# domerin0/rnn-speech

Measured on AMD Instinct MI355X. Metric: audio_frames_per_sec_train_3x512_lstm_ctc, higher is better.
Workload: dtype f32

## Files before the change

### include/amdspeech.h

```cpp
#ifndef AMDSPEECH_H
#define AMDSPEECH_H

#include <stddef.h>
#include <stdint.h>

#ifdef __cplusplus
extern "C" {
#endif

#define AMDSPEECH_OK 0
#define AMDSPEECH_EINVAL (-1)
#define AMDSPEECH_EHIP (-2)
#define AMDSPEECH_EUNSUPPORTED (-3)
#define AMDSPEECH_ETIMEOUT (-4)

int amdspeech_version(void);
const char* amdspeech_last_error(void);
int amdspeech_device_cu_count(void);

int amdspeech_linear_fwd(void* stream, const float* x, const float* w, const float* b,
                         float* y, int M, int K, int N);
int amdspeech_linear_bwd(void* stream, const float* x, const float* w, const float* dy,
                         float* dx, float* dw, float* db, int M, int K, int N);

// ... 29 lines not shown
                               const float* A, int lda, const float* B, int ldb,
                               float* C, int ldc, const float* bias, int accumulate, void* scratch, size_t scratch_bytes);
int amdspeech_gemm_bf16_packed_plan(int transA, int transB, int M, int N, int K, int lda, int ldb, amdspeech_gemm_plan_info* out);
int amdspeech_bf16_copy(void* stream, const float* src, long ld, long rows, int cols, int transpose, unsigned short* dst, long ldd,
                        float* colsum, unsigned short* plain);
int amdspeech_bf16_transpose(void* stream, const unsigned short* src, long rows, int cols, unsigned short* dst, long ldd);

int amdspeech_batchnorm_fwd(void* stream, const float* x, float* y, float* xhat,
                            float* inv_std, int T, int B, int H, float eps);
int amdspeech_batchnorm_bwd(void* stream, const float* dy, const float* xhat,
                            const float* inv_std, float* dx, int T, int B, int H);

int amdspeech_batchnorm_sum(void* stream, const float* x, const float* global_sum, int n_total, float* out,
                            int T, int B, int H);
int amdspeech_batchnorm_apply(void* stream, const float* x, const float* global_sum, const float* global_sq,
                              int n_total, float eps, float* y, float* xhat, float* inv_std, int T, int B, int H);
int amdspeech_batchnorm_bwd_sums(void* stream, const float* dy, const float* xhat, float* sums, int T, int B, int H);
int amdspeech_batchnorm_bwd_apply(void* stream, const float* dy, const float* xhat, const float* inv_std,
                                  const float* global_sums, int n_total, float* dx, int T, int B, int H);

typedef struct amdspeech_lstm_desc {
    int T, B, H, L;
    float keep_in, keep_out;
    uint64_t seed;
    int precision;
    int flags;
} amdspeech_lstm_desc;

enum { AMDSPEECH_LSTM_ARMED = 1, AMDSPEECH_LSTM_ARM_NEXT = 2, AMDSPEECH_LSTM_SAME_WS = 4, AMDSPEECH_LSTM_PER_DIAGONAL = 8,
       AMDSPEECH_LSTM_INJECT_TIMEOUT = 16 };

enum {
    AMDSPEECH_LSTM_WS_Z0 = 0,
    AMDSPEECH_LSTM_WS_ZTOP = 1,
    AMDSPEECH_LSTM_WS_DZTOP = 2,
    AMDSPEECH_LSTM_WS_DZ0 = 3,
    AMDSPEECH_LSTM_WS_HFINAL = 4,
    AMDSPEECH_LSTM_WS_CFINAL = 5,
    AMDSPEECH_LSTM_WS_GATES = 6
};
size_t amdspeech_lstm_workspace_bytes(const amdspeech_lstm_desc* d);
void* amdspeech_lstm_ws_ptr(const amdspeech_lstm_desc* d, void* ws, int which);

int amdspeech_lstm_workspace_release(void* stream, void* ws);

int amdspeech_lstm_beside_forward(void* stream, const void* ws);

int amdspeech_lstm_beside_tail(void* stream, const void* ws);

int amdspeech_lstm_fwd(void* stream, const amdspeech_lstm_desc* d, void* ws,
                       const float* kernels, long kernel_stride,
                       const float* biases, long bias_stride,
                       const int* lengths, const float* h0, const float* c0);
int amdspeech_lstm_pair_fusable(const amdspeech_lstm_desc* d);
int amdspeech_lstm_fwd_pair(void* stream, const amdspeech_lstm_desc* d_a, void* ws_a, const float* kernels_a, const float* biases_a,
                            const amdspeech_lstm_desc* d_b, void* ws_b, const float* kernels_b, const float* biases_b,
                            long kernel_stride, long bias_stride, const int* lengths, const float* h0_a, const float* c0_a);
int amdspeech_lstm_bwd_pair(void* stream, const amdspeech_lstm_desc* d_a, void* ws_a, const float* kernels_a, float* dkernels_a, float* dbiases_a,
                            const amdspeech_lstm_desc* d_b, void* ws_b, const float* kernels_b, float* dkernels_b, float* dbiases_b,
                            long kernel_stride, long bias_stride, const int* lengths);
int amdspeech_lstm_status(const amdspeech_lstm_desc* d, void* ws);
int amdspeech_lstm_bwd(void* stream, const amdspeech_lstm_desc* d, void* ws,
                       const float* kernels, long kernel_stride,
                       float* dkernels, float* dbiases, long bias_stride,
                       const int* lengths);

typedef struct amdspeech_ctc_head {
    const float* w_out;
    const float* b_out;
    float* logits;
    const int* dense_labels;
    float* loss;
    float* dlogits;
    void* ctc_ws;
    int C, U;
} amdspeech_ctc_head;
int amdspeech_lstm_ctc_fusable(const amdspeech_lstm_desc* d, int C, int U);
int amdspeech_lstm_fwd_ctc(void* stream, const amdspeech_lstm_desc* d, void* ws,
                           const float* kernels, long kernel_stride, const float* biases, long bias_stride,
                           const int* lengths, const float* h0, const float* c0, const amdspeech_ctc_head* head);
int amdspeech_lstm_bwd_ctc(void* stream, const amdspeech_lstm_desc* d, void* ws,
                           const float* kernels, long kernel_stride, float* dkernels, float* dbiases, long bias_stride,
                           const int* lengths, const amdspeech_ctc_head* head);

int amdspeech_lstm_dropout_multipliers(void* stream, const amdspeech_lstm_desc* d, int which, int layer, float* out);

enum { AMDSPEECH_LSTM_PATH_FLOW = 0, AMDSPEECH_LSTM_PATH_BIG1 = 1, AMDSPEECH_LSTM_PATH_BIG = 2, AMDSPEECH_LSTM_PATH_HOIST = 3,
       AMDSPEECH_LSTM_PATH_DIAG = 4, AMDSPEECH_LSTM_PATH_DIAG_BF3 = 5 };
typedef struct amdspeech_lstm_plan_info {
    int fwd_path, bwd_path, nmt, kb, mv, wpx, uw, fwd_mt, pair, bf16p, bf16p_reserved, xw_parts, nfw, w_pieces, dz0_inkernel, flow2_q;
} amdspeech_lstm_plan_info;
int amdspeech_lstm_plan(const amdspeech_lstm_desc* d, int C, int U, amdspeech_lstm_plan_info* out);
int amdspeech_lstm_plan_xw_halves(const amdspeech_lstm_desc* d, int C, int U);
int amdspeech_lstm_plan_xw_ksteps(const amdspeech_lstm_desc* d, int C, int U);

enum {
    AMDSPEECH_BIDIR_WS_Z0 = 0, AMDSPEECH_BIDIR_WS_YTOP_FW = 1, AMDSPEECH_BIDIR_WS_YTOP_BW = 2, AMDSPEECH_BIDIR_WS_DYTOP_FW = 3,
    AMDSPEECH_BIDIR_WS_DYTOP_BW = 4, AMDSPEECH_BIDIR_WS_DZ0 = 5, AMDSPEECH_BIDIR_WS_HFINAL = 6, AMDSPEECH_BIDIR_WS_CFINAL = 7
};
size_t amdspeech_lstm_bidir_workspace_bytes(const amdspeech_lstm_desc* d);
void* amdspeech_lstm_bidir_ws_ptr(const amdspeech_lstm_desc* d, void* ws, int which);
long amdspeech_lstm_bidir_layer_stride(const amdspeech_lstm_desc* d);
int amdspeech_lstm_bidir_path(const amdspeech_lstm_desc* d);
typedef struct amdspeech_lstm_bidir_plan_info {
    int path, cus, fwd_kpw, fwd_waves, fwd_groups, fwd_wgs, fwd_lds, bwd_kpw, bwd_waves, bwd_groups, bwd_wgs, bwd_lds;
} amdspeech_lstm_bidir_plan_info;
int amdspeech_lstm_bidir_plan(const amdspeech_lstm_desc* d, amdspeech_lstm_bidir_plan_info* out);
int amdspeech_lstm_bidir_fwd(void* stream, const amdspeech_lstm_desc* d, void* ws, const float* const* kernels,
                             const float* const* biases, const int* lengths, const float* h0, const float* c0);
int amdspeech_lstm_bidir_bwd(void* stream, const amdspeech_lstm_desc* d, void* ws, const float* const* kernels,
                             float* const* dkernels, float* const* dbiases, const int* lengths);
int amdspeech_lstm_bidir_status(const amdspeech_lstm_desc* d, void* ws);
int amdspeech_lstm_bidir_dropout_multipliers(void* stream, const amdspeech_lstm_desc* d, int dir, int which, int layer, float* out);

size_t amdspeech_ctc_workspace_bytes(int T, int B, int C, int U);
int amdspeech_ctc_loss_fwd_bwd(void* stream, const float* logits, const int* dense_labels,
                               const int* lengths, int T, int B, int C, int U,
                               float* loss, float* dlogits, void* ws);
int amdspeech_ctc_loss_fwd_bwd_staged(void* stream, const float* logits, const int* dense_labels,
                                      const int* lengths, int T, int B, int C, int U, float* loss,
                                      float* dlogits, void* ws, int stage);

enum { AMDSPEECH_CTC_KERNEL_WAVE = 0, AMDSPEECH_CTC_KERNEL_SHIFT = 1, AMDSPEECH_CTC_KERNEL_PAIR = 2, AMDSPEECH_CTC_KERNEL_EDGE = 3 };
typedef struct amdspeech_ctc_plan_info {
    int kernel, threads, rmax, smax;
} amdspeech_ctc_plan_info;
int amdspeech_ctc_plan(int T, int B, int C, int U, amdspeech_ctc_plan_info* out);

size_t amdspeech_ctc_align_workspace_bytes(int T, int B, int C, int U);
int amdspeech_ctc_align_plan(int T, int B, int C, int U, amdspeech_ctc_plan_info* out);
int amdspeech_ctc_align(void* stream, const float* logits, const int* dense_labels, const int* lengths,
                        int T, int B, int C, int U, int* frame_label, int* frame_state, int* spans,
                        float* score, float* confidence, void* ws);

int amdspeech_ctc_greedy_decode(void* stream, const float* logits, const int* lengths,
                                int T, int B, int C, int* ids, int* out_len, int* ws);

int amdspeech_merge_repeated(void* stream, int* ids, int* lens, int T, int B, int pad);

int amdspeech_edit_distance(void* stream, const int* a, const int* a_len, int lda, const int* b,
                            const int* b_len, int ldb, int n_pairs, int* out);

int amdspeech_ctc_beam_search_host(const float* logits, const int* lengths, int T, int B, int C,
                                   int beam_width, int merge_repeated, int* ids, int* out_len,
                                   float* log_prob);
int amdspeech_ctc_beam_search_host_mt(const float* logits, const int* lengths, int T, int B, int C,
                                      int beam_width, int merge_repeated, int* ids, int* out_len,
                                      float* log_prob, int max_threads);
int amdspeech_ctc_beam_search_host_nbest(const float* logits, const int* lengths, int T, int B, int C,
                                         int beam_width, int merge_repeated, int n_best, int* ids, int* out_len,
                                         float* log_prob, int* n_found, int max_threads);

int amdspeech_edit_distance_host(const int* a, const int* a_len, int lda, const int* b, const int* b_len, int ldb,
                                 int n_pairs, int* out);

uint32_t amdspeech_crc32c(const void* data, size_t n, uint32_t crc);

int amdspeech_audio_probe(const char* path, int* sample_rate, int* channels, long* frames);
int amdspeech_audio_decode(const char* path, float* out, long capacity, long* frames, int* sample_rate,
                           int verify);

size_t amdspeech_resample_workspace_bytes(int B);
int amdspeech_resample_num_samples(int n_samples, int rate_in, int rate_out);
int amdspeech_resample(void* stream, const float* pcm, const int* n_samples, int B, int n_max, int rate_in,
                       int rate_out, float* out, int out_max, void* ws);

// ... 149 lines not shown
```

### rnn-speech_amd/csrc/common.h

```cpp
#pragma once
#include <hip/hip_runtime.h>
#include <stdint.h>
#include <stdio.h>
#include <stdarg.h>
#include <mutex>

#include "../../include/amdspeech.h"

namespace amdspeech {

void set_error(const char* fmt, ...);

#define AS_CHECK_ARG(cond, ...)                         \
    do {                                                \
        if (!(cond)) {                                  \
            ::amdspeech::set_error(__VA_ARGS__);        \
            return AMDSPEECH_EINVAL;                    \
        }                                               \
    } while (0)

#define AS_CHECK_HIP(expr)                                                          \
    do {                                                                            \
        hipError_t e__ = (expr);                                                    \
        if (e__ != hipSuccess) {                                                    \
// ... 20 lines not shown
        first = (__atomic_load_n(seen, __ATOMIC_ACQUIRE) & bit) == 0;
    }
    explicit operator bool() const { return first; }
    void done() { if (bit) __atomic_fetch_or(seen, bit, __ATOMIC_RELEASE); }
};

int runtime_switch(const char* name, int dflt);
#ifdef AMDSPEECH_DEVTRACE
static inline int dev_knob(const char* name, int dflt) { return runtime_switch(name, dflt); }
const char* dev_knob_str(const char* name);
#else
static inline int dev_knob(const char*, int dflt) { return dflt; }
static inline const char* dev_knob_str(const char*) { return nullptr; }
#endif

static inline int ceil_div(long a, long b) { return (int)((a + b - 1) / b); }
static inline size_t align_up(size_t x, size_t a) { return (x + a - 1) / a * a; }

typedef float f32x4 __attribute__((ext_vector_type(4)));
typedef float f32x16 __attribute__((ext_vector_type(16)));

int gemm_f32(hipStream_t s, bool transA, bool transB, int M, int N, int K, const float* A, int lda,
             const float* B, int ldb, float* C, int ldc, const float* bias, bool accumulate,
             float* colsum = nullptr,
             const int* gate = nullptr, int gate_need = 0,
             unsigned* gate_err = nullptr);
typedef amdspeech_gemm_plan_info GemmPlan;
int gemm_f32_plan(bool transA, bool transB, int M, int N, int K, const float* A, int lda, const float* B, int ldb, const float* C,
                  int ldc, const float* bias, bool accumulate, bool colsum, bool gate, GemmPlan* out);
int gemm_f32_launch(hipStream_t s, const GemmPlan& p, bool transA, bool transB, int M, int N, int K, const float* A, int lda,
                    const float* B, int ldb, float* C, int ldc, const float* bias, bool accumulate, float* colsum = nullptr,
                    const int* gate = nullptr, int gate_need = 0, unsigned* gate_err = nullptr);
bool gemm_skinny_plan(bool transB, int M, int N, int K, const float* A, int lda, const float* B, int ldb, const float* C, int ldc,
                      const float* bias, GemmPlan* out);
int gemm_skinny_launch(hipStream_t s, const GemmPlan& p, bool transB, int M, int N, int K, const float* A, int lda, const float* B,
                       int ldb, float* C, int ldc, const float* bias, bool accumulate);
bool gemm_skinny_tn_plan(int M, int N, int K, const float* A, int lda, const float* B, int ldb, bool accumulate, bool colsum, GemmPlan* out);
int gemm_skinny_tn_launch(hipStream_t s, const GemmPlan& p, int M, int N, int K, const float* A, int lda, const float* B, int ldb,
                          float* C, int ldc, bool accumulate, float* colsum);
constexpr int GEMM_GROUP_MAX = AMDSPEECH_GEMM_GROUP_MAX;
int gemm_f32_tn_group(hipStream_t s, int count, int M, int N, int K, const float* const* A, int lda, const float* const* B,
                      int ldb, float* const* C, int ldc, float* const* colsum, bool accumulate,
                      const int* gate = nullptr, int gate_need = 0, unsigned* gate_err = nullptr);
bool gemm_f32_tn_group_ok(int M, int N, int K, const float* A, int lda, const float* B, int ldb);
int gemm_f32_tn_group_plan(int count, int M, int N, int K, const float* A, int lda, const float* B, int ldb, const float* C,
                           bool accumulate, GemmPlan* out);
int colsum_accumulate(hipStream_t s, const float* x, int rows, int cols, int ld, float* out);
int gemm_bf3(hipStream_t s, bool transA, bool transB, int M, int N, int K, const float* A, int lda, const float* B, int ldb,
             float* C, int ldc, const float* bias, bool accumulate);
int gemm_bf16(hipStream_t s, bool transA, bool transB, int M, int N, int K, const float* A, int lda, const float* B, int ldb,
              float* C, int ldc, const float* bias, bool accumulate);
int gemm_bf_plan(bool single, bool transA, bool transB, int M, int N, int K, const float* A, int lda, const float* B, int ldb,
                 const float* C, int ldc, const float* bias, bool accumulate, GemmPlan* out);

int bf16p_copy(hipStream_t s, const float* src, long ld, long rows, int cols, bool transpose, unsigned short* dst, long ldd, float* colsum,
               unsigned short* plain = nullptr);
size_t bf16p_partial_bytes(int M, int N, int K);
size_t bf16p_partial_bytes_max();
int bf16p_transpose(hipStream_t s, const unsigned short* src, long rows, int cols, unsigned short* dst, long ldd);
int bf16p_gemm(hipStream_t s, int M, int N, int K, const unsigned short* Ak, long lda, const unsigned short* Bk, long ldb, float* C, long ldc,
               const float* bias, bool accumulate, void* partial, size_t partial_bytes);
bool gemm_bf16_packed_ok(bool transA, bool transB, int M, int N, int K, int lda, int ldb);
size_t gemm_bf16_packed_scratch_bytes(int M, int N, int K);
int gemm_bf16_packed(hipStream_t s, bool transA, bool transB, int M, int N, int K, const float* A, int lda, const float* B, int ldb,
                     float* C, int ldc, const float* bias, bool accumulate, float* colsum, void* scratch, size_t scratch_bytes);

int ctc_prepare_targets(hipStream_t s, const int* dense_labels, const int* lengths, int T, int B, int C, int U, void* ws);

__host__ __device__ __forceinline__ uint32_t mix32(uint32_t x) {
    x ^= x >> 16; x *= 0x7feb352dU; x ^= x >> 15; x *= 0x846ca68bU; x ^= x >> 16;
    return x;
}
__device__ __forceinline__ float uniform01(uint64_t seed, uint32_t tensor, uint32_t idx) {
    uint32_t a = mix32(idx ^ (uint32_t)seed);
    uint32_t b = mix32(a + tensor * 0x9e3779b9U + (uint32_t)(seed >> 32));
    return (float)(b >> 8) * (1.0f / 16777216.0f);
}
__host__ __device__ __forceinline__ uint32_t random24(uint64_t seed, uint32_t stream, uint32_t idx) {
    uint32_t a = mix32(idx ^ (uint32_t)seed);
    uint32_t b = mix32(a + stream * 0x9e3779b9U + (uint32_t)(seed >> 32));
    return b >> 8;
}

}
```

### rnn-speech_amd/csrc/gemm_skinny.hip

```cpp
#include "common.h"
#include <string.h>

namespace amdspeech {

typedef __amdgpu_buffer_rsrc_t sk_rsrc_t;
typedef unsigned sk_u32x4 __attribute__((ext_vector_type(4)));

struct SkinnyArgs {
    const float* A; const float* B; float* C; const float* bias;
    int M, N, K, lda, ldb, ldc, accumulate;
};

constexpr unsigned SK_OOB = 0x80000000u;

__device__ __forceinline__ f32x4 sk_load4(sk_rsrc_t rs, unsigned byte_off) {
    const sk_u32x4 w = __builtin_amdgcn_raw_buffer_load_b128(rs, byte_off, 0, 0);
    f32x4 r;
    r.x = __uint_as_float(w.x); r.y = __uint_as_float(w.y); r.z = __uint_as_float(w.z); r.w = __uint_as_float(w.w);
    return r;
}
__device__ __forceinline__ float sk_load1(sk_rsrc_t rs, unsigned byte_off) {
    return __uint_as_float(__builtin_amdgcn_raw_buffer_load_b32(rs, byte_off, 0, 0));
}

struct SkinnyOut {
    sk_rsrc_t c, c_in, bias;
    __device__ __forceinline__ void init(const SkinnyArgs& g) {
        const unsigned cbytes = (unsigned)(((size_t)(g.M - 1) * g.ldc + g.N) * 4);
        c = __builtin_amdgcn_make_buffer_rsrc(g.C, 0, cbytes, 0x00020000);
        c_in = __builtin_amdgcn_make_buffer_rsrc(g.C, 0, g.accumulate ? cbytes : 0u, 0x00020000);
        bias = __builtin_amdgcn_make_buffer_rsrc(const_cast<float*>(g.bias), 0, g.bias != nullptr ? (unsigned)g.N * 4u : 0u, 0x00020000);
    }
    __device__ __forceinline__ unsigned offset(const SkinnyArgs& g, int row, int n) const {
        return (row < g.M && n < g.N) ? (unsigned)((size_t)row * g.ldc + n) * 4u : SK_OOB;
    }
    __device__ __forceinline__ f32x4 addend(const SkinnyArgs& g, unsigned off, int n) const {
        return sk_load4(bias, n < g.N ? (unsigned)n * 4u : SK_OOB) + sk_load4(c_in, off);
    }
    __device__ __forceinline__ void store(unsigned off, f32x4 v) const {
        sk_u32x4 w;
        w.x = __float_as_uint(v.x); w.y = __float_as_uint(v.y); w.z = __float_as_uint(v.z); w.w = __float_as_uint(v.w);
        __builtin_amdgcn_raw_buffer_store_b128(w, c, off, 0, 0);
    }
};

template <int NT>
__global__ __launch_bounds__(256) void gemm_skinny_n_kernel(SkinnyArgs g) {
    constexpr int KC = 64, LD = NT * 16 + ((NT & 1) ? 4 : 12);
    static_assert((4 * LD) % 32 == 16 && LD % 4 == 0, "bank spread");
    __shared__ __attribute__((aligned(16))) float wt[2][KC][LD];
    const int tid = threadIdx.x, w = tid >> 6, lane = tid & 63, m = lane & 15, kg = lane >> 4;
    const int row = blockIdx.x * 64 + w * 16 + m;
    const sk_rsrc_t ra = __builtin_amdgcn_make_buffer_rsrc(const_cast<float*>(g.A), 0, (unsigned)(((size_t)(g.M - 1) * g.lda + g.K) * 4), 0x00020000);
    const sk_rsrc_t rb = __builtin_amdgcn_make_buffer_rsrc(const_cast<float*>(g.B), 0, (unsigned)(((size_t)(g.K - 1) * g.ldb + g.N) * 4), 0x00020000);
    const int chunks = (g.K + KC - 1) / KC;

    f32x4 wreg[NT], a_cur[4], a_nxt[4];
    auto load_w = [&](int c) __attribute__((always_inline)) {
#pragma unroll
        for (int i = 0; i < NT; ++i) {
            const int slot = i * 256 + tid, k = slot / (4 * NT), n4 = slot % (4 * NT);
            const int kk = c * KC + k;
            const bool ok = n4 * 4 < g.N && kk < g.K;
            wreg[i] = sk_load4(rb, ok ? (unsigned)(kk * g.ldb + n4 * 4) * 4u : SK_OOB);
        }
    };
    auto put_w = [&](int buf) __attribute__((always_inline)) {
#pragma unroll
        for (int i = 0; i < NT; ++i) {
            const int slot = i * 256 + tid, k = slot / (4 * NT), n4 = slot % (4 * NT);
            *reinterpret_cast<f32x4*>(&wt[buf][k][n4 * 4]) = wreg[i];
        }
    };
    auto load_a = [&](int c, f32x4* a) __attribute__((always_inline)) {
#pragma unroll
        for (int s = 0; s < 4; ++s) {
            const int kk = c * KC + 16 * s + 4 * kg;
            const bool ok = row < g.M && kk < g.K;
            a[s] = sk_load4(ra, ok ? (unsigned)((size_t)row * g.lda + kk) * 4u : SK_OOB);
        }
    };

    f32x4 acc[NT];
#pragma unroll
    for (int i = 0; i < NT; ++i) acc[i] = f32x4{0.f, 0.f, 0.f, 0.f};
    load_w(0);
    load_a(0, a_cur);
    put_w(0);
    __syncthreads();
    for (int c = 0; c < chunks; ++c) {
        const int buf = c & 1;
        load_w(c + 1);
        load_a(c + 1, a_nxt);
        __builtin_amdgcn_sched_barrier(0);
        float bq[2][NT][4];
        auto read_b = [&](int s, float (*b)[4]) __attribute__((always_inline)) {
#pragma unroll
            for (int nt = 0; nt < NT; ++nt) {
                const float* col = &wt[buf][16 * s + 4 * kg][nt * 16 + m];
                b[nt][0] = col[0]; b[nt][1] = col[LD]; b[nt][2] = col[2 * LD]; b[nt][3] = col[3 * LD];
            }
        };
        read_b(0, bq[0]);
#pragma unroll
        for (int s = 0; s < 4; ++s) {
            if (s < 3) read_b(s + 1, bq[(s + 1) & 1]);
            __builtin_amdgcn_sched_barrier(0);
#pragma unroll
            for (int j = 0; j < 4; ++j)
#pragma unroll
                for (int nt = 0; nt < NT; ++nt)
                    acc[nt] = __builtin_amdgcn_mfma_f32_16x16x4f32(bq[s & 1][nt][j], a_cur[s][j], acc[nt], 0, 0, 0);
            __builtin_amdgcn_sched_barrier(0);
        }
        put_w(buf ^ 1);
#pragma unroll
        for (int s = 0; s < 4; ++s) a_cur[s] = a_nxt[s];
        __syncthreads();
    }
    SkinnyOut out;
    out.init(g);
    unsigned off[NT];
    f32x4 add[NT];
#pragma unroll
    for (int nt = 0; nt < NT; ++nt) {
        off[nt] = out.offset(g, row, nt * 16 + 4 * kg);
        add[nt] = out.addend(g, off[nt], nt * 16 + 4 * kg);
    }
#pragma unroll
    for (int nt = 0; nt < NT; ++nt) out.store(off[nt], acc[nt] + add[nt]);
}

template <int KT, bool B_KC>
__global__ __launch_bounds__(256) void gemm_skinny_k_kernel(SkinnyArgs g) {
    const int tid = threadIdx.x, w = tid >> 6, lane = tid & 63, m = lane & 15, kg = lane >> 4;
    const int row0 = blockIdx.x * 128 + w * 32;
    const sk_rsrc_t ra = __builtin_amdgcn_make_buffer_rsrc(const_cast<float*>(g.A), 0, (unsigned)(((size_t)(g.M - 1) * g.lda + g.K) * 4), 0x00020000);
    const size_t b_extent = B_KC ? (size_t)(g.N - 1) * g.ldb + g.K : (size_t)(g.K - 1) * g.ldb + g.N;
    const sk_rsrc_t rb = __builtin_amdgcn_make_buffer_rsrc(const_cast<float*>(g.B), 0, (unsigned)(b_extent * 4), 0x00020000);
    SkinnyOut out;
    out.init(g);

    f32x4 a[2][KT];
#pragma unroll
    for (int mt = 0; mt < 2; ++mt)
#pragma unroll
        for (int kt = 0; kt < KT; ++kt) {
            const int row = row0 + mt * 16 + m, kk = 16 * kt + 4 * kg;
            const bool ok = row < g.M && kk < g.K;
            a[mt][kt] = sk_load4(ra, ok ? (unsigned)((size_t)row * g.lda + kk) * 4u : SK_OOB);
        }
    struct Tile { f32x4 b[2][KT], bias[2], old[2][2]; unsigned off[2][2]; };
    auto fetch = [&](int nt, Tile& t) __attribute__((always_inline)) {
#pragma unroll
        for (int q = 0; q < 2; ++q) {
            const int n = (nt + q) * 16 + m;
#pragma unroll
            for (int kt = 0; kt < KT; ++kt) {
                const int kk = 16 * kt + 4 * kg;
                const bool ok = n < g.N && kk < g.K;
                if (B_KC) {
                    t.b[q][kt] = sk_load4(rb, ok ? (unsigned)(n * g.ldb + kk) * 4u : SK_OOB);
                } else {
                    const unsigned o = ok ? (unsigned)(kk * g.ldb + n) * 4u : SK_OOB;
                    const unsigned st = ok ? (unsigned)g.ldb * 4u : 0u;
                    t.b[q][kt].x = sk_load1(rb, o);
                    t.b[q][kt].y = sk_load1(rb, o + st);
                    t.b[q][kt].z = sk_load1(rb, o + 2 * st);
                    t.b[q][kt].w = sk_load1(rb, o + 3 * st);
                }
            }
            const int nc = (nt + q) * 16 + 4 * kg;
            t.bias[q] = sk_load4(out.bias, nc < g.N ? (unsigned)nc * 4u : SK_OOB);
#pragma unroll
            for (int mt = 0; mt < 2; ++mt) {
                t.off[mt][q] = out.offset(g, row0 + mt * 16 + m, nc);
                t.old[mt][q] = sk_load4(out.c_in, t.off[mt][q]);
            }
        }
    };
    auto tile = [&](int nt, const Tile& cur, Tile& nxt) __attribute__((always_inline)) {
        fetch(nt + 2, nxt);
        __builtin_amdgcn_sched_barrier(0);
        f32x4 acc[2][2];
#pragma unroll
        for (int mt = 0; mt < 2; ++mt)
#pragma unroll
            for (int q = 0; q < 2; ++q) acc[mt][q] = cur.bias[q] + cur.old[mt][q];
#pragma unroll
        for (int kt = 0; kt < KT; ++kt)
#pragma unroll
            for (int j = 0; j < 4; ++j)
#pragma unroll
                for (int mt = 0; mt < 2; ++mt)
#pragma unroll
                    for (int q = 0; q < 2; ++q)
                        acc[mt][q] = __builtin_amdgcn_mfma_f32_16x16x4f32(cur.b[q][kt][j], a[mt][kt][j], acc[mt][q], 0, 0, 0);
#pragma unroll
        for (int mt = 0; mt < 2; ++mt)
#pragma unroll
            for (int q = 0; q < 2; ++q) out.store(cur.off[mt][q], acc[mt][q]);
        __builtin_amdgcn_sched_barrier(0);
    };
    const int all_tiles = (g.N + 15) / 16;
    const int per = ((all_tiles + (int)gridDim.y - 1) / (int)gridDim.y + 1) & ~1;
    const int nt0 = (int)blockIdx.y * per, ntiles = min(all_tiles, nt0 + per);
    Tile t0, t1;
    fetch(nt0, t0);
    for (int nt = nt0; nt < ntiles; nt += 4) {
        tile(nt, t0, t1);
        if (nt + 2 >= ntiles) break;
        tile(nt + 2, t1, t0);
    }
}

#ifndef SKTN_DIAG
#define SKTN_DIAG 0
#endif
struct SkinnyTnArgs {
    const float* S; const float* W; float* C; float* colsum;
    int K, s, wide, lds, ldw, ldc;
    int chunk;
    int nslices;
    int small_is_a;
    int colsum_small;
};

template <int FULL, int RT>
__global__ __launch_bounds__(512) void gemm_skinny_tn_kernel(SkinnyTnArgs g) {
    constexpr int NTS = 4 * FULL + RT;
    constexpr int PD = NTS <= 4 ? 4 : 2;
    constexpr int SP = 64 * FULL + 16 * RT, LDR = 65;
    constexpr int NF = FULL > 0 ? FULL : 1, NR = RT > 0 ? RT : 1;
    extern __shared__ __attribute__((aligned(16))) float lds[];
    const int tid = threadIdx.x, w = tid >> 6, lane = tid & 63, i = lane & 15, kq = lane >> 4;
    const int v = blockIdx.x, xcd = v & 7, q = v >> 3;
    const int chunk_id = xcd + 8 * (q / g.nslices), slice = q % g.nslices;
    const int r0 = chunk_id * g.chunk;
    if (r0 >= g.K) return;
    const sk_rsrc_t rs = __builtin_amdgcn_make_buffer_rsrc(const_cast<float*>(g.S), 0, (unsigned)(((size_t)(g.K - 1) * g.lds + g.s) * 4), 0x00020000);
    const sk_rsrc_t rw = __builtin_amdgcn_make_buffer_rsrc(const_cast<float*>(g.W), 0, (unsigned)(((size_t)(g.K - 1) * g.ldw + g.wide) * 4), 0x00020000);

    const int wcol = slice * 64 + 4 * i;
    const bool w_ok = wcol < g.wide;
    const bool ones_wanted = g.colsum != nullptr && !g.colsum_small;
    const int rem = g.s - 64 * FULL;
    const int rcol = 64 * FULL + RT * i;
    bool r_valid[NR];
#pragma unroll
    for (int e = 0; e < NR; ++e) r_valid[e] = RT > 0 && rcol + e < g.s;
    const bool ones_lane = ones_wanted && RT > 0 && i == rem / NR;
    const int ones_e = rem % NR;
    const bool cs_small = g.colsum != nullptr && g.colsum_small && slice == 0;
    const int groups = g.chunk / 32;
    f32x4 smf[PD][NF], wd[PD];
    float smr[PD][NR];
    auto fetch = [&](int t, int p) __attribute__((always_inline)) {
        const int row = r0 + 4 * (8 * t + w) + kq;
        const bool r_ok = row < g.K && t < groups;
        wd[p] = sk_load4(rw, (r_ok && w_ok) ? (unsigned)((size_t)row * g.ldw + wcol) * 4u : SK_OOB);
#pragma unroll
        for (int b = 0; b < FULL; ++b) smf[p][b] = sk_load4(rs, r_ok ? (unsigned)((size_t)row * g.lds + 64 * b + 4 * i) * 4u : SK_OOB);
        if (RT > 0) {
            const unsigned off = (r_ok && r_valid[0]) ? (unsigned)((size_t)row * g.lds + rcol) * 4u : SK_OOB;
            if (RT == 1) {
                smr[p][0] = sk_load1(rs, off);
            } else if (RT == 2) {
                typedef unsigned u2 __attribute__((ext_vector_type(2)));
                const u2 x = __builtin_amdgcn_raw_buffer_load_b64(rs, off, 0, 0);
                smr[p][0] = __uint_as_float(x.x); smr[p][1 % NR] = __uint_as_float(x.y);
            } else if (RT == 3) {
                typedef unsigned u3 __attribute__((ext_vector_type(3)));
                const u3 x = __builtin_amdgcn_raw_buffer_load_b96(rs, off, 0, 0);
                smr[p][0] = __uint_as_float(x.x); smr[p][1 % NR] = __uint_as_float(x.y); smr[p][2 % NR] = __uint_as_float(x.z);
            } else {
                const f32x4 x = sk_load4(rs, off);
                smr[p][0] = x.x; smr[p][1 % NR] = x.y; smr[p][2 % NR] = x.z; smr[p][3 % NR] = x.w;
            }
        }
    };
// ... 183 lines not shown
    g.colsum_small = small_is_a ? 0 : 1;
    g.nslices = p.tiles_n;
    g.chunk = p.k_chunk;
    if (p.zero_fill) {
        const long n = (long)M * N;
        hipLaunchKernelGGL(skinny_zero_kernel, dim3(ceil_div(n, 256)), dim3(256), 0, st, C, M, N, ldc);
    }
    const dim3 grid(p.grid), block(512);
    const int full = p.variant / 8, rt = p.variant % 8;
    const size_t lds = (size_t)2 * (4 * full + rt) * 4 * 64 * 16;
#define SK_TN(F, R)                                                                                                          \
    do {                                                                                                                      \
        static unsigned long long seen = 0;                                                                                   \
        if (DeviceOnce once{&seen}) {                                                                                         \
            AS_CHECK_HIP(hipFuncSetAttribute(reinterpret_cast<const void*>(gemm_skinny_tn_kernel<F, R>),                      \
                                             hipFuncAttributeMaxDynamicSharedMemorySize, 2 * (4 * F + R) * 4 * 64 * 16));      \
            once.done();                                                                                                      \
        }                                                                                                                     \
        hipLaunchKernelGGL((gemm_skinny_tn_kernel<F, R>), grid, block, lds, st, g);                                           \
    } while (0)
    switch (p.variant) {
        case 1: SK_TN(0, 1); break;
        case 2: SK_TN(0, 2); break;
        case 3: SK_TN(0, 3); break;
        case 4: SK_TN(0, 4); break;
        case 8: SK_TN(1, 0); break;
        case 9: SK_TN(1, 1); break;
        case 10: SK_TN(1, 2); break;
        case 11: SK_TN(1, 3); break;
        case 12: SK_TN(1, 4); break;
        default: AS_CHECK_ARG(false, "gemm_skinny_tn: no kernel for variant %d", p.variant);
    }
#undef SK_TN
    AS_CHECK_LAUNCH();
    return AMDSPEECH_OK;
}

bool gemm_skinny_plan(bool transB, int M, int N, int K, const float* A, int lda, const float* B, int ldb, const float* C, int ldc,
                      const float* bias, GemmPlan* out) {
    static const bool enabled = dev_knob("AMDSPEECH_GEMM_SKINNY", 1) != 0;
    if (!enabled || M < 256) return false;
    if ((N | K | lda | ldb | ldc) & 3) return false;
    if (!aligned16(A) || !aligned16(B) || !aligned16(C) || (bias != nullptr && !aligned16(bias))) return false;
    const size_t lim = (size_t)SK_OOB;
    if (((size_t)(M - 1) * lda + K) * 4 >= lim) return false;
    if (((size_t)(M - 1) * ldc + N) * 4 >= lim) return false;
    GemmPlan p;
    memset(&p, 0, sizeof(p));
    p.splits = 1; p.col_slices = 1; p.k_chunk = K; p.a_vec = p.b_vec = 1; p.tiles_n = 1;
    if (K <= 80 && N >= 64) {
        const size_t be = transB ? (size_t)(N - 1) * ldb + K : (size_t)(K - 1) * ldb + N;
        if (be * 4 >= lim) return false;
        const int row_blocks = ceil_div(M, 128);
        const int kt = ceil_div(K, 16);
        p.family = AMDSPEECH_GEMM_SKINNY_K; p.variant = (kt <= 3 ? 3 : 5) * 2 + (transB ? 1 : 0);
        p.tiles_m = row_blocks;
        p.col_slices = (row_blocks < 512 && N >= 256 && kt <= 3) ? 2 : 1;
        p.grid = row_blocks * p.col_slices;
        *out = p;
        return true;
    }
    if (!transB && N <= 96 && K >= 64) {
        if (((size_t)(K - 1) * ldb + N) * 4 >= lim) return false;
        const int nt = ceil_div(N, 16);
        p.family = AMDSPEECH_GEMM_SKINNY_N; p.variant = nt < 6 ? nt : 6;
        p.tiles_m = ceil_div(M, 64);
        p.grid = p.tiles_m;
        *out = p;
        return true;
    }
    return false;
}

int gemm_skinny_launch(hipStream_t s, const GemmPlan& p, bool transB, int M, int N, int K, const float* A, int lda, const float* B,
                       int ldb, float* C, int ldc, const float* bias, bool accumulate) {
    SkinnyArgs g;
    g.A = A; g.B = B; g.C = C; g.bias = bias; g.M = M; g.N = N; g.K = K; g.lda = lda; g.ldb = ldb; g.ldc = ldc;
    g.accumulate = accumulate ? 1 : 0;
    const dim3 block(256);
    if (p.family == AMDSPEECH_GEMM_SKINNY_K) {
        const dim3 grid(p.tiles_m, p.col_slices);
#define SK_K(KT)                                                                                           \
        do {                                                                                               \
            if (transB) hipLaunchKernelGGL((gemm_skinny_k_kernel<KT, true>), grid, block, 0, s, g);        \
            else hipLaunchKernelGGL((gemm_skinny_k_kernel<KT, false>), grid, block, 0, s, g);              \
        } while (0)
        if (p.variant / 2 == 3) SK_K(3);
        else SK_K(5);
#undef SK_K
    } else {
        const dim3 grid(p.grid);
        switch (p.variant) {
            case 1: hipLaunchKernelGGL(gemm_skinny_n_kernel<1>, grid, block, 0, s, g); break;
            case 2: hipLaunchKernelGGL(gemm_skinny_n_kernel<2>, grid, block, 0, s, g); break;
            case 3: hipLaunchKernelGGL(gemm_skinny_n_kernel<3>, grid, block, 0, s, g); break;
            case 4: hipLaunchKernelGGL(gemm_skinny_n_kernel<4>, grid, block, 0, s, g); break;
            case 5: hipLaunchKernelGGL(gemm_skinny_n_kernel<5>, grid, block, 0, s, g); break;
            default: hipLaunchKernelGGL(gemm_skinny_n_kernel<6>, grid, block, 0, s, g); break;
        }
    }
    AS_CHECK_LAUNCH();
    return AMDSPEECH_OK;
}

}
```

### rnn-speech_amd/csrc/lstm.hip

```cpp
#include "common.h"
#include "gemm_core.h"
#include "ctc_core.h"
#include <stdlib.h>
#include <string.h>
#include <type_traits>
#include <mutex>
#include <unordered_map>

namespace amdspeech {

#define FLOW_WEIGHTS_RESIDENT() __builtin_amdgcn_s_waitcnt(0x0F70)
static unsigned long long* dev_trace_ptr() {
#ifdef AMDSPEECH_DEVTRACE
    if (const char* e = dev_knob_str("AMDSPEECH_TRACE_PTR")) return reinterpret_cast<unsigned long long*>(strtoull(e, nullptr, 0));
#endif
    return nullptr;
}
#ifndef BIG_WEIGHTS_RESIDENT
#define BIG_WEIGHTS_RESIDENT 1
#endif

struct LstmLayout {
    size_t wp, wq, z, hs, cs, gates, dg, dztop, dz0, dc, xp0, xp, hp, dgp, sync, xph, hph, dxh, prec, pdown, xwp, bigring, wopack, bfs, total;
    size_t fwd_set = 0;
// ... 19 lines not shown
    const long groups = (long)d->L * ((d->B + 15) / 16);
    return fwd_workers_fit(d) && fwd_worker_wgs_per_xcd(d, 4) <= 32 - FWD2_WORKER_RESERVE &&
           (size_t)d->T * groups * (d->H / 16) * 6144 < (1ull << 32);
}
static bool bf16p_layout_reserved(const amdspeech_lstm_desc* d) {
    static const int env = runtime_switch("AMDSPEECH_BF16_PACKED", 1);
    return env != 0 && d->precision == 2 && d->H == 1024;
}
static bool bf16p_layout_on(const amdspeech_lstm_desc* d) {
    return bf16p_layout_reserved(d) && ((long)d->T * d->B) % 64 == 0 && (long)d->T * d->B >= 256;
}
struct Bf16pBufs { unsigned short *zb, *wtb, *dgb, *wb, *zht, *dgt; char* partial; size_t partial_bytes; };
static size_t bf16p_scratch_floats(const amdspeech_lstm_desc* d) {
    const size_t TB = ((size_t)d->T * d->B + 63) / 64 * 64, H = d->H;
    const size_t bytes = TB * H * 2 + 4 * H * H * 2 + TB * 4 * H * 2 + H * 4 * H * 2 + 2 * H * TB * 2 + 4 * H * TB * 2 +
                         bf16p_partial_bytes_max() + 8 * 256;
    return (bytes + 3) / 4;
}
static Bf16pBufs bf16p_bufs(const amdspeech_lstm_desc* d, float* base) {
    const size_t TB = (size_t)d->T * d->B, H = d->H;
    char* p = reinterpret_cast<char*>(base);
    auto take = [&](size_t bytes) { char* r = p; p += align_up(bytes, 256); return r; };
    Bf16pBufs b;
    b.zb = reinterpret_cast<unsigned short*>(take(TB * H * 2));
    b.wtb = reinterpret_cast<unsigned short*>(take(4 * H * H * 2));
    b.dgb = reinterpret_cast<unsigned short*>(take(TB * 4 * H * 2));
    b.wb = reinterpret_cast<unsigned short*>(take(H * 4 * H * 2));
    b.zht = reinterpret_cast<unsigned short*>(take(2 * H * TB * 2));
    b.dgt = reinterpret_cast<unsigned short*>(take(4 * H * TB * 2));
    b.partial_bytes = bf16p_partial_bytes_max();
    b.partial = take(b.partial_bytes);
    return b;
}
static int bf16p_xw(hipStream_t s, const Bf16pBufs& b, int rows, int H, const float* Z, const float* K, float* G, const float* bias) {
    if (int rc = bf16p_copy(s, Z, H, rows, H, false, b.zb, H, nullptr)) return rc;
    if (int rc = bf16p_copy(s, K, 4 * H, H, 4 * H, true, b.wtb, H, nullptr)) return rc;
    return bf16p_gemm(s, rows, 4 * H, H, b.zb, H, b.wtb, H, G, 4 * H, bias, false, b.partial, b.partial_bytes);
}
static int bf16p_dx(hipStream_t s, const Bf16pBufs& b, int rows, int H, const float* dG, const float* K, float* dX) {
    if (int rc = bf16p_copy(s, dG, 4 * H, rows, 4 * H, false, b.dgb, 4 * H, nullptr)) return rc;
    if (int rc = bf16p_copy(s, K, 4 * H, H, 4 * H, false, b.wb, 4 * H, nullptr)) return rc;
    return bf16p_gemm(s, rows, H, 4 * H, b.dgb, 4 * H, b.wb, 4 * H, dX, H, nullptr, false, b.partial, b.partial_bytes);
}
static int bf16p_layer_bwd(hipStream_t s, const Bf16pBufs& b, int rows, int H, const float* Z, const float* Hp, const float* dG, const float* K,
                           float* dX, float* dK, float* dbias) {
    if (int rc = bf16p_copy(s, dG, 4 * H, rows, 4 * H, true, b.dgt, rows, dbias, b.dgb)) return rc;
    if (int rc = bf16p_copy(s, K, 4 * H, H, 4 * H, false, b.wb, 4 * H, nullptr)) return rc;
    if (int rc = bf16p_gemm(s, rows, H, 4 * H, b.dgb, 4 * H, b.wb, 4 * H, dX, H, nullptr, false, b.partial, b.partial_bytes)) return rc;
    if (int rc = bf16p_copy(s, Z, H, rows, H, true, b.zht, rows, nullptr)) return rc;
    if (int rc = bf16p_copy(s, Hp, H, rows, H, true, b.zht + (size_t)H * rows, rows, nullptr)) return rc;
    return bf16p_gemm(s, 2 * H, 4 * H, rows, b.zht, rows, b.dgt, rows, dK, 4 * H, nullptr, true, b.partial, b.partial_bytes);
}
static int bf16p_layer_bwd_copied(hipStream_t s, const Bf16pBufs& b, int rows, int H, const float* Z, const float* Hp, const float* K,
                                  float* dX, float* dK) {
    if (int rc = bf16p_copy(s, K, 4 * H, H, 4 * H, false, b.wb, 4 * H, nullptr)) return rc;
    if (int rc = bf16p_gemm(s, rows, H, 4 * H, b.dgb, 4 * H, b.wb, 4 * H, dX, H, nullptr, false, b.partial, b.partial_bytes)) return rc;
    if (int rc = bf16p_copy(s, Z, H, rows, H, true, b.zht, rows, nullptr)) return rc;
    if (int rc = bf16p_copy(s, Hp, H, rows, H, true, b.zht + (size_t)H * rows, rows, nullptr)) return rc;
    if (int rc = bf16p_transpose(s, b.dgb, rows, 4 * H, b.dgt, rows)) return rc;
    return bf16p_gemm(s, 2 * H, 4 * H, rows, b.zht, rows, b.dgt, rows, dK, 4 * H, nullptr, true, b.partial, b.partial_bytes);
}
static int bf16p_dk(hipStream_t s, const Bf16pBufs& b, int rows, int H, const float* Z, const float* Hp, const float* dG, float* dK, float* dbias) {
    if (int rc = bf16p_copy(s, Z, H, rows, H, true, b.zht, rows, nullptr)) return rc;
    if (int rc = bf16p_copy(s, Hp, H, rows, H, true, b.zht + (size_t)H * rows, rows, nullptr)) return rc;
    if (int rc = bf16p_copy(s, dG, 4 * H, rows, 4 * H, true, b.dgt, rows, dbias)) return rc;
    return bf16p_gemm(s, 2 * H, 4 * H, rows, b.zht, rows, b.dgt, rows, dK, 4 * H, nullptr, true, b.partial, b.partial_bytes);
}

static int check_desc(const amdspeech_lstm_desc* d) {
    AS_CHECK_ARG(d != nullptr, "lstm: null descriptor");
    AS_CHECK_ARG(d->T > 0 && d->B > 0 && d->H > 0 && d->L > 0, "lstm: bad shape T=%d B=%d H=%d L=%d",
                 d->T, d->B, d->H, d->L);
    AS_CHECK_ARG(d->H % 16 == 0, "lstm: hidden size %d must be a multiple of 16", d->H);
    AS_CHECK_ARG(d->keep_in > 0.f && d->keep_in <= 1.f && d->keep_out > 0.f && d->keep_out <= 1.f,
                 "lstm: keep probabilities must be in (0,1]");
    AS_CHECK_ARG((size_t)d->T * d->B * d->H < (1ull << 32), "lstm: T*B*H too large for the dropout counter");
    AS_CHECK_ARG(d->precision == 0 || ((d->precision == 1 || d->precision == 2) && d->H % 32 == 0),
                 "lstm: precision %d unsupported (0 = f32; 1 = bf16x3, 2 = bf16: both need H %% 32 == 0, H = %d)", d->precision, d->H);
    AS_CHECK_ARG((d->flags & ~(AMDSPEECH_LSTM_ARMED | AMDSPEECH_LSTM_ARM_NEXT | AMDSPEECH_LSTM_SAME_WS | AMDSPEECH_LSTM_PER_DIAGONAL |
                               AMDSPEECH_LSTM_INJECT_TIMEOUT)) == 0, "lstm: unknown flags 0x%x", d->flags);
    return AMDSPEECH_OK;
}

struct DropCfg { float keep_in, keep_out; uint64_t seed; int L; };

__device__ __forceinline__ float zmult(const DropCfg& c, int lp, uint32_t idx) {
    float m = 1.0f;
    if (c.keep_in < 1.0f && lp < c.L)
        m *= (uniform01(c.seed, 2u * lp, idx) < c.keep_in) ? (1.0f / c.keep_in) : 0.0f;
    if (c.keep_out < 1.0f && lp >= 1)
        m *= (uniform01(c.seed, 2u * (lp - 1) + 1u, idx) < c.keep_out) ? (1.0f / c.keep_out) : 0.0f;
    return m;
}

__global__ void apply_zmult_kernel(float* x, long n, DropCfg c, int lp) {
    long i = (long)blockIdx.x * blockDim.x + threadIdx.x;
    if (i < n) x[i] *= zmult(c, lp, (uint32_t)i);
}

__global__ void pack_fwd_kernel(const float* __restrict__ kernels, long kstride, float* __restrict__ wp,
                                int H, int L, int UW, int grouped) {
    const int NT = UW / 4, NKB = 2 * H / 16, NUB = H / UW;
    const long total = (long)L * 2 * H * 4 * H;
    long o = (long)blockIdx.x * blockDim.x + threadIdx.x;
    if (o >= total) return;
    int m = o & 3, lane = (o >> 2) & 63;
    long r = o >> 8;
    int nt = r % NT; r /= NT;
    int kb = r % NKB; r /= NKB;
    int ub = r % NUB; int l = r / NUB;
    int j = lane & 15, kq = lane >> 4;
    int c = nt * 16 + j, g = c / UW, u = c % UW;
    if (grouped) { g = j >> 2; u = nt * 4 + (j & 3); }
    int k = kb * 16 + 4 * kq + m;
    wp[o] = kernels[l * kstride + (long)k * 4 * H + g * H + ub * UW + u];
}

__global__ void pack_bwd_kernel(const float* __restrict__ kernels, long kstride, float* __restrict__ wq,
                                int H, int L) {
    const int NRB = 2 * H / 16, NKB = 4 * H / 16;
    const long total = (long)L * 2 * H * 4 * H;
    long o = (long)blockIdx.x * blockDim.x + threadIdx.x;
    if (o >= total) return;
    int m = o & 3, lane = (o >> 2) & 63;
    long r = o >> 8;
    int kb = r % NKB; r /= NKB;
    int rb = r % NRB; int l = r / NRB;
    int row = rb * 16 + (lane & 15), col = kb * 16 + 4 * (lane >> 4) + m;
    wq[o] = kernels[l * kstride + (long)row * 4 * H + col];
}

__device__ __forceinline__ size_t packed_off(int row, int k, int K) {
    return ((((size_t)(row >> 4) * (K >> 4) + (k >> 4)) * 64) + (((k >> 2) & 3) * 16 + (row & 15))) * 4 + (k & 3);
}

__global__ void pack_rows_kernel(const float* __restrict__ src, size_t src_stride, float* __restrict__ dst,
                                 int B, int K, int nmat) {
    const size_t per = (size_t)B * K;
    const size_t i = (size_t)blockIdx.x * blockDim.x + threadIdx.x;
    if (i >= per * nmat) return;
    const int mat = i / per;
    const size_t r = i % per;
    const int row = r / K, k = r % K;
    const size_t bpk = (size_t)((B + 15) / 16 * 16) * K;
    dst[(size_t)mat * bpk + packed_off(row, k, K)] = src[(size_t)mat * src_stride + r];
}

__global__ __launch_bounds__(256) void mask_pack_rows_kernel(float* __restrict__ z, float* __restrict__ dst, int B, int K, int T,
                                                             DropCfg c, int masked) {
    const size_t per4 = (size_t)B * K / 4;
    const size_t i = (size_t)blockIdx.x * blockDim.x + threadIdx.x;
    if (i >= per4 * T) return;
    const int t = i / per4;
    const size_t r = (i % per4) * 4;
    const int row = r / K, k = r % K;
    const size_t e = (size_t)t * B * K + r;
    float4 v = *reinterpret_cast<const float4*>(z + e);
    if (masked) {
        v.x *= zmult(c, 0, (uint32_t)e); v.y *= zmult(c, 0, (uint32_t)(e + 1));
        v.z *= zmult(c, 0, (uint32_t)(e + 2)); v.w *= zmult(c, 0, (uint32_t)(e + 3));
        *reinterpret_cast<float4*>(z + e) = v;
    }
    const size_t bpk = (size_t)((B + 15) / 16 * 16) * K;
    *reinterpret_cast<float4*>(dst + (size_t)t * bpk + packed_off(row, k, K)) = v;
}

__global__ __launch_bounds__(256) void flow_fwd_prepare_kernel(const float* __restrict__ h0, const float* __restrict__ c0,
                                                               float* __restrict__ hs, float* __restrict__ cs,
                                                               float* __restrict__ hph, unsigned* __restrict__ sync_words,
                                                               int T, int B, int H, int L) {
    const int bp = (B + 15) / 16 * 16;
    const size_t per = (size_t)bp * H;
    const size_t i = (size_t)blockIdx.x * blockDim.x + threadIdx.x;
    if (i < 40) sync_words[i] = 0u;
    if (i >= per * L) return;
    const int l = i / per;
    const size_t r = i % per;
    const int row = r / H, k = r % H;
    float hv = 0.f;
    if (row < B) {
        const size_t e = (size_t)row * H + k, bh = (size_t)B * H;
        hv = h0 ? h0[l * bh + e] : 0.f;
        hs[(size_t)l * (T + 1) * bh + e] = hv;
        cs[(size_t)l * (T + 1) * bh + e] = c0 ? c0[l * bh + e] : 0.f;
    }
    hph[(size_t)l * (T + 1) * per + packed_off(row, k, H)] = hv;
}

__device__ __forceinline__ float sigmoidf_(float x) { return 1.0f / (1.0f + expf(-x)); }

#include "lstm_step_fwd.h"
#include "lstm_flow.h"
}
#include "ctc_flow.h"
namespace amdspeech {

#include "lstm_flow_fwd.h"
#include "lstm_big_fwd.h"
#include "lstm_step_bwd.h"
#include "lstm_flow_bwd.h"
#include "lstm_big_bwd.h"
#include "lstm_step_bf3.h"
constexpr int PROF_SEGS = 16;
static bool g_prof_on = false;
static hipEvent_t g_prof_ev[2][PROF_SEGS][2];
static int g_prof_launches[2] = {0, 0};
static int g_prof_nseg[2] = {0, 0};
static bool g_prof_valid[2] = {false, false};
static double g_prof_flops[2][2] = {{0, 0}, {0, 0}};
static void prof_flops(int which, double recurrence, double other) { g_prof_flops[which][0] = recurrence; g_prof_flops[which][1] = other; }

static void prof_begin(int which, hipStream_t s, int seg = 0) {
    if (g_prof_on && seg < PROF_SEGS) (void)hipEventRecord(g_prof_ev[which][seg][0], s);
}
static void prof_end(int which, hipStream_t s, int launches, int seg = 0) {
    if (!g_prof_on || seg >= PROF_SEGS) return;
    (void)hipEventRecord(g_prof_ev[which][seg][1], s);
    g_prof_launches[which] = launches;
    g_prof_nseg[which] = seg + 1;
    g_prof_valid[which] = true;
}

static hipStream_t g_side = nullptr;
static hipEvent_t g_fork = nullptr;
static int side_stream_init() {
    if (g_side) return AMDSPEECH_OK;
    AS_CHECK_HIP(hipStreamCreateWithFlags(&g_side, hipStreamNonBlocking));
    AS_CHECK_HIP(hipEventCreateWithFlags(&g_fork, hipEventDisableTiming));
    return AMDSPEECH_OK;
}
static hipStream_t g_chain = nullptr, g_gemm = nullptr;
static hipEvent_t g_ev_a = nullptr, g_ev_b = nullptr, g_ev_c = nullptr;
static int g_overlap_state = 0;
static int overlap_init() {
    if (g_overlap_state != 0) return g_overlap_state;
    g_overlap_state = -1;
    int dev = 0, cus = 0;
    if (hipGetDevice(&dev) != hipSuccess) return -1;
    if (hipDeviceGetAttribute(&cus, hipDeviceAttributeMultiprocessorCount, dev) != hipSuccess || cus != 256) return -1;
    uint32_t chain_mask[8] = {0, 0, ~0u, ~0u, ~0u, ~0u, ~0u, ~0u}, gemm_mask[8] = {~0u, ~0u, 0, 0, 0, 0, 0, 0};
    if (hipExtStreamCreateWithCUMask(&g_chain, 8, chain_mask) != hipSuccess) return -1;
    if (hipExtStreamCreateWithCUMask(&g_gemm, 8, gemm_mask) != hipSuccess) return -1;
    if (hipEventCreateWithFlags(&g_ev_a, hipEventDisableTiming) != hipSuccess) return -1;
    if (hipEventCreateWithFlags(&g_ev_b, hipEventDisableTiming) != hipSuccess) return -1;
    if (hipEventCreateWithFlags(&g_ev_c, hipEventDisableTiming) != hipSuccess) return -1;
    g_overlap_state = 1;
    return 1;
}
constexpr int DK_CHUNKS = 8, DK_SIDE = 5;

static int gemm_reduced(const amdspeech_lstm_desc* d, hipStream_t s, bool ta, bool tb, int M, int N, int K, const float* A, int lda,
                        const float* B, int ldb, float* C, int ldc, const float* bias, bool accumulate) {
    return (d->precision == 2 ? gemm_bf16 : gemm_bf3)(s, ta, tb, M, N, K, A, lda, B, ldb, C, ldc, bias, accumulate);
}
static int gemm_batched(const amdspeech_lstm_desc* d, hipStream_t s, bool ta, bool tb, int M, int N, int K, const float* A, int lda,
                        const float* B, int ldb, float* C, int ldc, const float* bias, bool accumulate) {
    if (d->precision != 0) return gemm_reduced(d, s, ta, tb, M, N, K, A, lda, B, ldb, C, ldc, bias, accumulate);
    return gemm_f32(s, ta, tb, M, N, K, A, lda, B, ldb, C, ldc, bias, accumulate);
}
static int pick_uw(const amdspeech_lstm_desc* d) {
    const long wgs8 = (long)d->L * (d->H / 8) * ceil_div(d->B, 32);
    return (d->H % 8 == 0 && wgs8 >= 96) ? 8 : 4;
}

static int device_cus() {
    static int cus = -1;
    if (cus < 0) {
        int dev = 0;
        if (hipGetDevice(&dev) != hipSuccess ||
            hipDeviceGetAttribute(&cus, hipDeviceAttributeMultiprocessorCount, dev) != hipSuccess) cus = 0;
    }
    return cus;
}

static bool use_big_fwd(const amdspeech_lstm_desc* d) {
    static const int env = runtime_switch("AMDSPEECH_BIG", 1);
    return env != 0 && !(d->flags & AMDSPEECH_LSTM_PER_DIAGONAL) && d->precision >= 0 && d->precision <= 2 && d->H == 1024 &&
           (d->B + 15) / 16 <= 4 && device_cus() == 256 &&
           (size_t)2 * ((d->B + 15) / 16 * 16) * d->H * 4 < (1ull << 32);
}

static bool use_flow(const amdspeech_lstm_desc* d) {
    static const int env = runtime_switch("AMDSPEECH_FLOW", 1);
    return env != 0 && !(d->flags & AMDSPEECH_LSTM_PER_DIAGONAL) && flow_shape_ok(d) && device_cus() == 256 && d->L * ((d->B + 15) / 16) <= 8;
}

template <bool CF>
static void (*flow_fwd_kernel(int kb, int pr, int mv, int mh, int me))(FlowArgs) {
    switch (kb) {
        case 1: return lstm_fwd_flow2<1, 0, 0, CF>;
        case 2: return pr == 2 ? lstm_fwd_flow2<2, 2, 0, CF> : (pr == 1 ? lstm_fwd_flow2<2, 1, 0, CF> : lstm_fwd_flow2<2, 0, 0, CF>);
        case 3: return lstm_fwd_flow2<3, 0, 0, CF>;
        default:
            if (pr == 0 && mv == 1 && mh == 1) return me > 0 ? lstm_fwd_flow2<4, 0, 1, CF, 1, FWD2_HALF_KSTEPS> : lstm_fwd_flow2<4, 0, 1, CF, 1>;
            if (pr == 0 && mv == 1) return lstm_fwd_flow2<4, 0, 1, CF>;
            return pr == 2 ? lstm_fwd_flow2<4, 2, 0, CF> : (pr == 1 ? lstm_fwd_flow2<4, 1, 0, CF> : lstm_fwd_flow2<4, 0, 0, CF>);
    }
}
template <bool CF>
static void (*flow_bwd_kernel(int kb, int pr))(FlowBwdArgs) {
    if (pr == 2) return kb == 2 ? lstm_bwd_flow2<2, 2, CF> : lstm_bwd_flow2<4, 2, CF>;
    if (pr == 1) return kb == 2 ? lstm_bwd_flow2<2, 1, CF> : lstm_bwd_flow2<4, 1, CF>;
    return kb == 1 ? lstm_bwd_flow2<1, 0, CF> : (kb == 2 ? lstm_bwd_flow2<2, 0, CF> : (kb == 3 ? lstm_bwd_flow2<3, 0, CF> : lstm_bwd_flow2<4, 0, CF>));
}
static int flow_fill_fwd_panels(hipStream_t s, const amdspeech_lstm_desc* d, float* ws, const LstmLayout& lo, int set) {
    const size_t bph = (size_t)(d->B + 15) / 16 * 16 * d->H;
    float* base = ws + (size_t)set * lo.fwd_set;
    AS_CHECK_HIP(hipMemsetD32Async(reinterpret_cast<hipDeviceptr_t>(base + lo.xph + (size_t)d->T * bph), (int)FLOW_SENTINEL,
                                   (size_t)d->L * d->T * bph, s));
    AS_CHECK_HIP(hipMemsetD32Async(reinterpret_cast<hipDeviceptr_t>(base + lo.hph), (int)FLOW_SENTINEL, (size_t)d->L * (d->T + 1) * bph, s));
    return AMDSPEECH_OK;
}
static int flow_fill_bwd_panels(hipStream_t s, const amdspeech_lstm_desc* d, float* ws, const LstmLayout& lo, bool ctc_head = false) {
    const size_t bpg = (size_t)((d->B + 15) / 16) * 16 * 4 * d->H;
    AS_CHECK_HIP(hipMemsetAsync(ws + lo.prec, 0, (lo.total - lo.prec) * sizeof(float), s));
    if (ctc_head)
        AS_CHECK_HIP(hipMemsetD32Async(reinterpret_cast<hipDeviceptr_t>(ws + lo.dztop), (int)FLOW_SENTINEL, (size_t)d->T * d->B * d->H, s));
    if (d->L > 1)
        AS_CHECK_HIP(hipMemsetD32Async(reinterpret_cast<hipDeviceptr_t>(ws + lo.dxh), (int)FLOW_SENTINEL,
                                       (size_t)(d->L - 1) * d->T * (bpg / 4), s));
    return AMDSPEECH_OK;
}
struct ArmState {
    hipEvent_t join = nullptr; bool pending = false;
    hipEvent_t pre = nullptr; int idle_xcds = 0;
    hipEvent_t post = nullptr; int post_flags = 0;
    int clean_set = 0;
    int xw_par = -1;
    int xw_cover = 0;
    long xw_key = 0;
};
static std::mutex g_arm_mutex;
static std::unordered_map<const void*, ArmState> g_arm;
static int flow_xw_parity(hipStream_t s, const void* ws, bool trust, long key, float* xwp, size_t frame_floats, int T, unsigned* par) {
    std::lock_guard<std::mutex> lock(g_arm_mutex);
    ArmState& st = g_arm[ws];
    if (trust && st.xw_par >= 0 && st.xw_key == key) {
        const int old = st.xw_par;
        if (T > st.xw_cover)
            AS_CHECK_HIP(hipMemsetD32Async(reinterpret_cast<hipDeviceptr_t>(xwp + (size_t)st.xw_cover * frame_floats), old,
                                           (size_t)(T - st.xw_cover) * frame_floats, s));
        st.xw_par = old ^ 1;
    } else {
        AS_CHECK_HIP(hipMemsetAsync(xwp, 0, (size_t)T * frame_floats * sizeof(float), s));
        st.xw_par = 1;
    }
    st.xw_cover = T; st.xw_key = key;
    *par = (unsigned)st.xw_par;
    return AMDSPEECH_OK;
}
static void flow_xw_forget(const void* ws) {
    std::lock_guard<std::mutex> lock(g_arm_mutex);
    auto it = g_arm.find(ws);
    if (it != g_arm.end()) it->second.xw_par = -1;
}
static int flow_arm_fork(hipStream_t s) {
    if (int rc = side_stream_init()) return rc;
    AS_CHECK_HIP(hipEventRecord(g_fork, s));
    AS_CHECK_HIP(hipStreamWaitEvent(g_side, g_fork, 0));
    return AMDSPEECH_OK;
}
static int flow_clean_set(const void* ws) {
    std::lock_guard<std::mutex> lock(g_arm_mutex);
    auto it = g_arm.find(ws);
    return it == g_arm.end() ? 0 : it->second.clean_set;
}
static int flow_arm_publish(const void* ws, int clean_set) {
    std::lock_guard<std::mutex> lock(g_arm_mutex);
    ArmState& st = g_arm[ws];
    st.clean_set = clean_set;
    if (!st.join) AS_CHECK_HIP(hipEventCreateWithFlags(&st.join, hipEventDisableTiming));
    AS_CHECK_HIP(hipEventRecord(st.join, g_side));
    st.pending = true;
    return AMDSPEECH_OK;
}
static int flow_arm_settle(hipStream_t s, const void* ws) {
    std::lock_guard<std::mutex> lock(g_arm_mutex);
    auto it = g_arm.find(ws);
    if (it == g_arm.end() || !it->second.pending) return AMDSPEECH_OK;
    AS_CHECK_HIP(hipStreamWaitEvent(s, it->second.join, 0));
    it->second.pending = false;
    return AMDSPEECH_OK;
}
static int flow_arm_release(hipStream_t s, const void* ws) {
    std::lock_guard<std::mutex> lock(g_arm_mutex);
    auto it = g_arm.find(ws);
    if (it == g_arm.end()) return AMDSPEECH_OK;
    if (it->second.pending) AS_CHECK_HIP(hipStreamWaitEvent(s, it->second.join, 0));
    if (it->second.join) (void)hipEventDestroy(it->second.join);
    if (it->second.pre) (void)hipEventDestroy(it->second.pre);
    if (it->second.post) (void)hipEventDestroy(it->second.post);
    g_arm.erase(it);
    return AMDSPEECH_OK;
}
static int flow_mark_postlaunch(hipStream_t s, const void* ws, int flags) {
    std::lock_guard<std::mutex> lock(g_arm_mutex);
    ArmState& st = g_arm[ws];
    st.post_flags = flags;
    if (flags == 0) return AMDSPEECH_OK;
    if (!st.post) AS_CHECK_HIP(hipEventCreateWithFlags(&st.post, hipEventDisableTiming));
    AS_CHECK_HIP(hipEventRecord(st.post, s));
    return AMDSPEECH_OK;
}
static int flow_mark_prelaunch(hipStream_t s, const void* ws, int idle_xcds) {
    std::lock_guard<std::mutex> lock(g_arm_mutex);
    ArmState& st = g_arm[ws];
    st.idle_xcds = idle_xcds;
    if (idle_xcds <= 0) return AMDSPEECH_OK;
    if (!st.pre) AS_CHECK_HIP(hipEventCreateWithFlags(&st.pre, hipEventDisableTiming));
    AS_CHECK_HIP(hipEventRecord(st.pre, s));
    return AMDSPEECH_OK;
}

static int ctc_head_nfw(const amdspeech_lstm_desc* d, int C, int U, int wpx) {
    static const int env = runtime_switch("AMDSPEECH_FLOW_CTC", 1);
    if (env == 0) return 0;
    const int groups = d->L * ((d->B + 15) / 16), spare = 8 - groups, smax = 2 * U + 1;
    if (spare < 1 || C < 16 || C > 16 * CF_NTC || C % 16 != 0 || U < 1 || smax > 384 || d->H % 64 != 0) return 0;
    if ((size_t)d->B * d->T * smax * 4 >= (1ull << 31) || (size_t)d->T * d->B * d->H * 4 >= (1ull << 31)) return 0;
    int nfw = 32 - wpx < 4 ? 32 - wpx : 4;
    if (nfw < 1 || d->B > spare * nfw * 2 * 2) return 0;
    return nfw;
}
static CtcFlow ctc_head_args(const amdspeech_lstm_desc* d, const amdspeech_ctc_head* h, float* ws, const LstmLayout& lo, float* panels, int nfw) {
    const CtcLayout cl = ctc_layout(d->T, d->B, h->C, h->U);
    char* w = static_cast<char*>(h->ctc_ws);
    CtcFlow c;
    c.on = 1; c.C = h->C; c.smax = cl.smax; c.nfw = nfw; c.T = d->T; c.B = d->B;
    c.ztp = panels ? panels + lo.xph + (size_t)d->L * d->T * ((size_t)(d->B + 15) / 16 * 16 * d->H) : nullptr;
    c.wo = h->w_out; c.wo_pack = ws + lo.wopack; c.bo = h->b_out;
    c.logits = h->logits; c.logp = reinterpret_cast<float*>(w + cl.logp); c.alpha = reinterpret_cast<float*>(w + cl.alpha);
    c.ll = reinterpret_cast<float*>(w + cl.ll); c.loss = h->loss; c.dlogits = h->dlogits; c.dztop = ws + lo.dztop;
    c.ext = reinterpret_cast<const int*>(w + cl.ext); c.slen = reinterpret_cast<const int*>(w + cl.slen);
    c.valid = reinterpret_cast<const int*>(w + cl.valid);
    return c;
}

enum class Path {
    flow,
    big1,
    big,
    hoist,
    diag,
    diag_bf3,
};
struct LstmPlan {
    amdspeech_lstm_desc d;
    int nmt;
    bool flow_shape;
    int xw_parts;
    int xw_half;
    bool big_ring;
    bool bf16p_reserved;
    bool bf16p;
    Path fwd, bwd;
    bool pair;
    int uw;
    unsigned long long limit;
    void (*fwd_diag)(FwdArgs); int fwd_mt;
    void (*bwd_diag)(BwdArgs);
    void (*fwd_big)(BigFwdArgs); void (*bwd_big)(BigBwdArgs);
    void (*fwd_flow)(FlowArgs); void (*bwd_flow)(FlowBwdArgs);
    size_t fwd_lds, bwd_lds;
    int mv, wpx, wpw;
    int mh;
    int me;
    int nfw;
    int dz0_inkernel;
    int w_pieces, w_t0, w_dz0;
    bool w_deal;
};

// ... 48 lines not shown
    static const int workers_env = runtime_switch("AMDSPEECH_FLOW_FWD_WORKERS", 3);
    const int groups = L * p.nmt, spare = 8 - groups;
    p.wpw = 8;
    if (workers_env != 0 && p.xw_parts > 0)
        for (int waves = 4; waves <= 8 && p.mv == 0; waves += 4) {
            const int per = fwd_worker_wgs_per_xcd(d, waves);
            if (per <= 32 - FWD2_WORKER_RESERVE) { p.mv = 1; p.wpx = per; p.wpw = waves; }
        }
    p.mh = (workers_env != 1 && p.mv == 1 && p.wpw == 4 && p.xw_half > 0) ? 1 : 0;
    p.me = (p.mh == 1 && workers_env != 2) ? FWD2_HALF_KSTEPS : 0;
    if (head != nullptr) p.nfw = ctc_head_nfw(d, head->C, head->U, p.wpx);
    const int kb = H / 128;
    p.fwd_flow = head != nullptr ? flow_fwd_kernel<true>(kb, pr, p.mv, p.mh, p.me) : flow_fwd_kernel<false>(kb, pr, p.mv, p.mh, p.me);
    p.bwd_flow = head != nullptr ? flow_bwd_kernel<true>(kb, pr) : flow_bwd_kernel<false>(kb, pr);
    p.fwd_lds = head != nullptr ? (size_t)2 * CF_FOLLOW_TEAM_FLOATS * sizeof(float) : 0;
    p.bwd_lds = ((size_t)2 * 1024 + 2 * 8 * 256 + (FLOW2_WINDOW ? 2 : 1) * 8 * kb * 256 + (size_t)(flow2_q(kb, pr) - 1) * 1024) * sizeof(float);
    const size_t lds_workers = (size_t)2 * 2 * 2 * BK * LDS_LD * sizeof(float);
    if (p.bwd_lds < lds_workers) p.bwd_lds = lds_workers;
    if (p.bwd_lds < (size_t)2 * CF_LEAD_TEAM_FLOATS * sizeof(float)) p.bwd_lds = (size_t)2 * CF_LEAD_TEAM_FLOATS * sizeof(float);

    const FlowGemmShare g = flow_gemm_share();
    const bool workers = g.pieces > 0 && g.percent > 0 && T >= 64 && groups < 8 && H % 128 == 0;
    const int share = g.set ? g.percent : (pr != 0 ? (head != nullptr ? g.percent / 2 - 1 : g.percent * 3 / 4) : g.percent);
    static const int dz0_in = runtime_switch("AMDSPEECH_FLOW_DZ0", 1);
    p.dz0_inkernel = dz0_in ? 1 : 0;
    p.w_dz0 = (p.dz0_inkernel || workers) ? 0 : 1;
    p.w_pieces = workers ? g.pieces : 0;
    static const int deal = runtime_switch("AMDSPEECH_FLOW_WORKER_DEAL", -1);
    p.w_deal = workers && g.pieces <= 8 && (deal > 0 || (deal < 0 && head != nullptr));
    p.w_t0 = workers ? T - (int)((long)T * share / 100) : T;
    if (p.w_t0 < 2) p.w_t0 = 2;
    return p;
}

static LstmLayout lstm_layout(const LstmPlan& p) {
    const size_t T = p.d.T, B = p.d.B, H = p.d.H, L = p.d.L;
    const size_t tbh = T * B * H;
    LstmLayout o;
    size_t off = 0;
    auto take = [&](size_t n) { size_t r = off; off += (n + 63) / 64 * 64; return r; };
    o.xwp = 0;
    if (p.xw_parts > 0) o.xwp = take(T * L * ((B + 15) / 16) * (H / 16) * (p.xw_parts * 1024 + p.xw_half * 512));
    o.wp = take(L * 2 * H * 4 * H);
    o.wq = take(L * 2 * H * 4 * H);
    o.z = take((L + 1) * tbh);
    o.hs = take(L * (T + 1) * B * H);
    o.cs = take(L * (T + 1) * B * H);
    o.gates = take(L * tbh * 4);
    o.dg = take(L * tbh * 4);
    o.dztop = take(tbh);
    o.dz0 = take(tbh);
    o.dc = take(L * 2 * B * H);
    const size_t bp = (B + 15) / 16 * 16;
    o.xp0 = take(T * bp * H);
    o.xp = take(L * 2 * bp * H);
    o.hp = take(L * 2 * bp * H);
    o.dgp = take(L * 2 * bp * 4 * H);
    o.sync = take(64);
    o.xph = o.hph = o.dxh = o.prec = o.pdown = o.wopack = off;
    if (p.flow_shape) {
        o.xph = take((L + 1) * T * bp * H);
        o.hph = take(L * (T + 1) * bp * H);
        o.fwd_set = off - o.xph;
        take((L + 1) * T * bp * H);
        take(L * (T + 1) * bp * H);
        o.wopack = take((H / 16) * CF_NTC * 256);
        o.dxh = take(L * T * bp * H);
        const size_t slot = (size_t)L * (bp / 16) * (H / 16) * (H / 16) * 256;
        o.prec = take(2 * slot);
        o.pdown = take(4 * L * (bp / 16) * (H / 16) * (H / 128) * 256);
        take(L * (bp / 16) * 2 * (H / 16) * 1024);
    }
    o.bigring = off;
    if (p.big_ring) o.bigring = take((size_t)2 * (bp / 16) * (2 * 32 * 32 * 256 + 64 * 1024));
    o.bfs = off;
    if (p.bf16p_reserved) o.bfs = take(bf16p_scratch_floats(&p.d));
    o.total = off;
    return o;
}

struct FwdCall {
    const amdspeech_lstm_desc* d; float* ws; const float* kernels; long kstride; const float* biases; long bstride;
    const int* lengths; const float* h0; const float* c0; const amdspeech_ctc_head* head;
    LstmPlan p; LstmLayout lo;
};
struct BwdCall {
    const amdspeech_lstm_desc* d; float* ws; const float* kernels; long kstride; float* dkernels; float* dbiases; long bstride;
    const int* lengths; const amdspeech_ctc_head* head;
    LstmPlan p; LstmLayout lo;
};
static DropCfg drop_cfg(const amdspeech_lstm_desc* d) { return DropCfg{d->keep_in, d->keep_out, d->seed, d->L}; }
static int mask_dz0(hipStream_t s, const BwdCall& c) {
    if (c.d->keep_in < 1.0f) {
        const long n = (long)c.d->T * c.d->B * c.d->H;
        hipLaunchKernelGGL(apply_zmult_kernel, dim3(ceil_div(n, 256)), dim3(256), 0, s, c.ws + c.lo.dz0, n, drop_cfg(c.d), 0);
        AS_CHECK_LAUNCH();
    }
    return AMDSPEECH_OK;
}

static int fwd_prologue(hipStream_t s, FwdCall& c) {
    const amdspeech_lstm_desc* d = c.d;
    if (int rc = check_desc(d)) return rc;
    AS_CHECK_ARG(c.ws && c.kernels && c.biases && c.lengths, "lstm_fwd: null pointer");
    AS_CHECK_ARG(((uintptr_t)c.ws % 256) == 0, "lstm_fwd: workspace must be 256-byte aligned");
    if (int rc = flow_arm_settle(s, c.ws)) return rc;
    if (int rc = flow_mark_prelaunch(s, c.ws, 0)) return rc;
    c.p = lstm_plan(d, c.head);
    c.lo = lstm_layout(c.p);
    AS_CHECK_ARG(c.head == nullptr || c.p.fwd == Path::flow, "lstm_fwd_ctc: the fused CTC head needs the whole-sequence kernels (amdspeech_lstm_ctc_fusable)");
    prof_flops(0, 0.0, 0.0);
    AS_CHECK_HIP(hipMemsetAsync(c.ws + c.lo.sync, 0, 64, s));
    const long wtotal = (long)d->L * 2 * d->H * 4 * d->H;
    if (c.p.fwd == Path::diag_bf3)
        hipLaunchKernelGGL(pack_fwd_bf3_kernel, dim3(ceil_div(wtotal, 256)), dim3(256), 0, s, c.kernels, c.kstride,
                           reinterpret_cast<unsigned short*>(c.ws + c.lo.wp), d->H, d->L);
    else
        hipLaunchKernelGGL(pack_fwd_kernel, dim3(ceil_div(wtotal, 256)), dim3(256), 0, s, c.kernels, c.kstride,
                           c.ws + c.lo.wp, d->H, d->L, c.p.uw, 0);
    AS_CHECK_LAUNCH();
    return AMDSPEECH_OK;
}
static int fwd_stage(hipStream_t s, const FwdCall& c) {
    const amdspeech_lstm_desc* d = c.d;
    const int T = d->T, B = d->B, H = d->H, L = d->L;
    float* ws = c.ws;
    const LstmLayout& lo = c.lo;
    const size_t bh = (size_t)B * H, bp = (size_t)(B + 15) / 16 * 16, n0 = (size_t)T * bh;
    for (int l = 0; l < L; ++l) {
        float* hs0 = ws + lo.hs + (size_t)l * (T + 1) * bh;
        float* cs0 = ws + lo.cs + (size_t)l * (T + 1) * bh;
        if (c.h0) AS_CHECK_HIP(hipMemcpyAsync(hs0, c.h0 + l * bh, bh * 4, hipMemcpyDeviceToDevice, s));
        else AS_CHECK_HIP(hipMemsetAsync(hs0, 0, bh * 4, s));
        if (c.c0) AS_CHECK_HIP(hipMemcpyAsync(cs0, c.c0 + l * bh, bh * 4, hipMemcpyDeviceToDevice, s));
        else AS_CHECK_HIP(hipMemsetAsync(cs0, 0, bh * 4, s));
    }
    if (d->keep_in < 1.0f) {
        hipLaunchKernelGGL(apply_zmult_kernel, dim3(ceil_div(n0, 256)), dim3(256), 0, s, ws + lo.z, (long)n0, drop_cfg(d), 0);
        AS_CHECK_LAUNCH();
    }
    if (c.p.fwd == Path::diag_bf3) {
        hipLaunchKernelGGL(pack_rows_bf3_kernel, dim3(ceil_div(n0, 256)), dim3(256), 0, s, ws + lo.z, bh,
                           reinterpret_cast<unsigned short*>(ws + lo.xp0), B, H, T);
        for (int l = 0; l < L; ++l)
            hipLaunchKernelGGL(pack_rows_bf3_kernel, dim3(ceil_div(bh, 256)), dim3(256), 0, s,
                               ws + lo.hs + (size_t)l * (T + 1) * bh, bh,
                               reinterpret_cast<unsigned short*>(ws + lo.hp + ((size_t)l * 2 + (l & 1)) * bp * H), B, H, 1);
    } else {
        const bool diag = c.p.fwd == Path::diag;
        if (diag)
            hipLaunchKernelGGL(pack_rows_kernel, dim3(ceil_div(n0, 256)), dim3(256), 0, s, ws + lo.z, bh, ws + lo.xp0, B, H, T);
        for (int l = 0; l < L; ++l)
            hipLaunchKernelGGL(pack_rows_kernel, dim3(ceil_div(bh, 256)), dim3(256), 0, s,
                               ws + lo.hs + (size_t)l * (T + 1) * bh, bh, ws + lo.hp + ((size_t)l * 2 + (diag ? (l & 1) : 0)) * bp * H,
                               B, H, 1);
    }
    AS_CHECK_LAUNCH();
    return AMDSPEECH_OK;
}

static int fwd_flow(hipStream_t s, const FwdCall& c) {
    const amdspeech_lstm_desc* d = c.d;
    const LstmPlan& p = c.p;
    const LstmLayout& lo = c.lo;
    float* ws = c.ws;
    const int T = d->T, B = d->B, H = d->H, L = d->L;
    const size_t bp = (size_t)(B + 15) / 16 * 16, bph = bp * H, bh = (size_t)B * H;
    const DropCfg dc = drop_cfg(d);
    unsigned* err = reinterpret_cast<unsigned*>(ws + lo.sync);
    const int set = (d->flags & AMDSPEECH_LSTM_ARMED) ? flow_clean_set(ws) : 0;
    if (!(d->flags & AMDSPEECH_LSTM_ARMED))
        if (int rc = flow_fill_fwd_panels(s, d, ws, lo, set)) return rc;
    float* const panels = ws + (size_t)set * lo.fwd_set;
    hipLaunchKernelGGL(flow_fwd_prepare_kernel, dim3(ceil_div((long)L * bph, 256)), dim3(256), 0, s, c.h0, c.c0, ws + lo.hs, ws + lo.cs,
                       panels + lo.hph, err, T, B, H, L);
    hipLaunchKernelGGL(mask_pack_rows_kernel, dim3(ceil_div((long)T * bh / 4, 256)), dim3(256), 0, s, ws + lo.z, ws + lo.xp0, B, H, T,
                       dc, d->keep_in < 1.0f ? 1 : 0);
    AS_CHECK_LAUNCH();
    FlowArgs fa;
    fa.wp = ws + lo.wp; fa.bias = c.biases; fa.bias_stride = c.bstride;
    fa.z = ws + lo.z; fa.hs = ws + lo.hs; fa.cs = ws + lo.cs; fa.gates = ws + lo.gates; fa.lengths = c.lengths;
    fa.xp0 = ws + lo.xp0; fa.xph = panels + lo.xph; fa.hph = panels + lo.hph; fa.err = err;
    fa.T = T; fa.B = B; fa.H = H; fa.L = L; fa.drop = dc;
    fa.limit = p.limit;
    fa.trace = dev_trace_ptr(); fa.trace_layer = dev_knob("AMDSPEECH_TRACE_LAYER", L > 1 ? 1 : 0);
    fa.tickets = err + 16;
    fa.xwp = ws + lo.xwp; fa.xw_par = 0u; fa.w_wpx = p.wpx; fa.w_wpw = p.wpw;
    if (p.mv > 0)
        if (int rc = flow_xw_parity(s, ws, (d->flags & (AMDSPEECH_LSTM_ARMED | AMDSPEECH_LSTM_SAME_WS)) != 0,
                                    (((long)B * 4096 + H) * 64 + L) * 8 + p.mv * 2 + p.mh, fa.xwp,
                                    (size_t)L * (bp / 16) * (H / 16) * (p.mv * 1024 + p.mh * 512), T,
                                    &fa.xw_par)) return rc;
    fa.cf = CtcFlow{}; fa.cf_on = 0; fa.cf_nfw = 0;
    if (c.head != nullptr) {
        const amdspeech_ctc_head* head = c.head;
        AS_CHECK_ARG(p.nfw > 0, "lstm_fwd_ctc: this shape does not take the fused CTC head (amdspeech_lstm_ctc_fusable)");
        fa.cf = ctc_head_args(d, head, ws, lo, panels, p.nfw); fa.cf_on = 1; fa.cf_nfw = p.nfw;
        fa.cf.lengths = c.lengths; fa.cf.err = err; fa.cf.limit = fa.limit;
        if (int rc = ctc_prepare_targets(s, head->dense_labels, c.lengths, T, B, head->C, head->U, head->ctc_ws)) return rc;
        hipLaunchKernelGGL(ctc_pack_wo_kernel, dim3(ceil_div((H / 16) * CF_NTC * 64, 256)), dim3(256), 0, s, head->w_out, ws + lo.wopack, H, head->C);
        AS_CHECK_LAUNCH();
        AS_CHECK_HIP(hipFuncSetAttribute(reinterpret_cast<const void*>(p.fwd_flow), hipFuncAttributeMaxDynamicSharedMemorySize, (int)p.fwd_lds));
    }
    prof_begin(0, s);
    const bool arm = (d->flags & AMDSPEECH_LSTM_ARM_NEXT) != 0;
    if (arm)
        if (int rc = flow_arm_fork(s)) return rc;
    if (int rc = flow_mark_prelaunch(s, ws, (p.mv > 0 && c.head == nullptr) ? 0 : 8 - L * p.nmt)) return rc;
    hipLaunchKernelGGL(p.fwd_flow, dim3(256), dim3(512), p.fwd_lds, s, fa);
    prof_end(0, s, T + L - 1);
    prof_flops(0, (double)T * L * 2.0 * B * 2 * H * 4 * H, 0.0);
    AS_CHECK_LAUNCH();
    if (arm) {
        if (int rc = flow_fill_bwd_panels(g_side, d, ws, lo, c.head != nullptr)) return rc;
        const long wtotal = (long)L * 2 * H * 4 * H;
        hipLaunchKernelGGL(pack_bwd_kernel, dim3(ceil_div(wtotal, 256)), dim3(256), 0, g_side, c.kernels, c.kstride, ws + lo.wq, H, L);
        AS_CHECK_LAUNCH();
        if (int rc = flow_fill_fwd_panels(g_side, d, ws, lo, 1 - set)) return rc;
        if (int rc = flow_arm_publish(ws, 1 - set)) return rc;
    }
    return AMDSPEECH_OK;
}

static int big_fwd_layers(hipStream_t s, int n, const FwdCall* st, bool big1) {
    const amdspeech_lstm_desc* d = st[0].d;
    const int T = d->T, B = d->B, H = d->H, L = d->L, nmt = ceil_div(B, 16);
    const size_t TB = (size_t)T * B, bp = (size_t)nmt * 16, bh = (size_t)B * H;
    if (big1) {
        static const hipError_t once = hipFuncSetAttribute(reinterpret_cast<const void*>(lstm_fwd_big1), hipFuncAttributeMaxDynamicSharedMemorySize, BIG1_LDS_BYTES);
        AS_CHECK_HIP(once);
    }
    BigFwd1Args b1;
    b1.n = n;
    for (int k = 0; k < n; ++k) {
        const FwdCall& q = st[k];
        unsigned* err = reinterpret_cast<unsigned*>(q.ws + q.lo.sync);
        BigFwdArgs& ba = b1.b[k];
        ba.wp = q.ws + q.lo.wp; ba.z = q.ws + q.lo.z; ba.hs = q.ws + q.lo.hs; ba.cs = q.ws + q.lo.cs; ba.gates = q.ws + q.lo.gates;
        ba.lengths = q.lengths;
        ba.err = err; ba.tickets = err + 16;
        ba.T = T; ba.B = B; ba.H = H; ba.L = L; ba.drop = drop_cfg(q.d);
        ba.limit = q.p.limit;
    }
    if (n == 1) b1.b[1] = b1.b[0];
    for (int l = 0; l < L; ++l) {
        for (int k = 0; k < n; ++k) {
            const FwdCall& q = st[k];
            float* ws = q.ws;
            const LstmLayout& lk = q.lo;
            const float* z = ws + lk.z + (size_t)l * TB * H;
            float* g = ws + lk.gates + (size_t)l * TB * 4 * H;
            if (int rc = q.p.bf16p ? bf16p_xw(s, bf16p_bufs(q.d, ws + lk.bfs), (int)TB, H, z, q.kernels + l * q.kstride, g, q.biases + l * q.bstride)
                                   : gemm_batched(q.d, s, false, false, (int)TB, 4 * H, H, z, H, q.kernels + l * q.kstride, 4 * H, g, 4 * H,
                                                  q.biases + l * q.bstride, false)) return rc;
            float* ring = ws + lk.hp + (size_t)l * 2 * bp * H;
            AS_CHECK_HIP(hipMemsetAsync(ring, 0, 2 * bp * H * sizeof(float), s));
            hipLaunchKernelGGL(pack_rows_kernel, dim3(ceil_div(bh, 256)), dim3(256), 0, s,
                               ws + lk.hs + (size_t)l * (T + 1) * bh, bh, ring, B, H, 1);
            hipLaunchKernelGGL(tag_panel_kernel, dim3(ceil_div(bp * H, 256)), dim3(256), 0, s, ring, bp * H, 1u);
            AS_CHECK_HIP(hipMemsetAsync(b1.b[k].tickets, 0, 8 * sizeof(unsigned), s));
            b1.b[k].hring = ring; b1.b[k].layer = l;
        }
        if (n == 1) b1.b[1] = b1.b[0];
        prof_begin(0, s, l);
        if (big1) hipLaunchKernelGGL(lstm_fwd_big1, dim3(256), dim3(512), BIG1_LDS_BYTES, s, b1);
        else hipLaunchKernelGGL(st[0].p.fwd_big, dim3(256), dim3(512), 0, s, b1.b[0]);
        prof_end(0, s, T * L, l);
    }
    AS_CHECK_LAUNCH();
    return AMDSPEECH_OK;
}
static int fwd_big(hipStream_t s, const FwdCall& c) {
    if (int rc = fwd_stage(s, c)) return rc;
    return big_fwd_layers(s, 1, &c, c.p.fwd == Path::big1);
}

static int fwd_diag(hipStream_t s, const FwdCall& c) {
    if (int rc = fwd_stage(s, c)) return rc;
    const amdspeech_lstm_desc* d = c.d;
    const int T = d->T, H = d->H, L = d->L;
    float* ws = c.ws;
    const LstmLayout& lo = c.lo;
    FwdArgs a;
    a.xp0 = ws + lo.xp0; a.xp = ws + lo.xp; a.hp = ws + lo.hp;
    a.wp = ws + lo.wp; a.bias = c.biases; a.bias_stride = c.bstride;
    a.z = ws + lo.z; a.hs = ws + lo.hs; a.cs = ws + lo.cs; a.gates = ws + lo.gates; a.lengths = c.lengths;
    a.T = T; a.B = d->B; a.H = H; a.L = L; a.drop = drop_cfg(d);
    a.hoist = 0; a.l0 = 0; a.mt0 = 0; a.dbg = 0;
    a.trace = dev_trace_ptr(); a.trace_d = a.trace ? dev_knob("AMDSPEECH_TRACE_D", T / 2) : -1;
    const dim3 grid = c.p.fwd == Path::diag_bf3 ? dim3(H / 8, L, ceil_div(c.p.nmt, 2)) : dim3(H / c.p.uw, L, c.p.nmt / c.p.fwd_mt);
    prof_begin(0, s);
    for (int dd = 0; dd < T + L - 1; ++dd) {
        a.d = dd;
        hipLaunchKernelGGL(c.p.fwd_diag, grid, dim3(8 * 64), 0, s, a);
    }
    prof_end(0, s, T + L - 1);
    AS_CHECK_LAUNCH();
    return AMDSPEECH_OK;
}

static int lstm_fwd(hipStream_t s, FwdCall c) {
    if (int rc = fwd_prologue(s, c)) return rc;
    switch (c.p.fwd) {
        case Path::flow: return fwd_flow(s, c);
        case Path::big: case Path::big1: return fwd_big(s, c);
        default: return fwd_diag(s, c);
    }
}

static int bwd_prologue(hipStream_t s, BwdCall& c) {
    const amdspeech_lstm_desc* d = c.d;
    if (int rc = check_desc(d)) return rc;
    AS_CHECK_ARG(c.ws && c.kernels && c.dkernels && c.dbiases && c.lengths, "lstm_bwd: null pointer");
    if (int rc = flow_arm_settle(s, c.ws)) return rc;
    if (int rc = flow_mark_postlaunch(s, c.ws, 0)) return rc;
    c.p = lstm_plan(d, c.head);
    c.lo = lstm_layout(c.p);
    const long wtotal = (long)d->L * 2 * d->H * 4 * d->H;
    if (c.p.bwd == Path::diag_bf3)
        hipLaunchKernelGGL(pack_bwd_bf3_kernel, dim3(ceil_div(wtotal, 256)), dim3(256), 0, s, c.kernels, c.kstride,
                           reinterpret_cast<unsigned short*>(c.ws + c.lo.wq), d->H, d->L);
    else if (!(c.p.bwd == Path::flow && (d->flags & AMDSPEECH_LSTM_ARMED)))
        hipLaunchKernelGGL(pack_bwd_kernel, dim3(ceil_div(wtotal, 256)), dim3(256), 0, s, c.kernels, c.kstride, c.ws + c.lo.wq, d->H, d->L);
    AS_CHECK_LAUNCH();
    AS_CHECK_ARG(c.head == nullptr || c.p.bwd == Path::flow, "lstm_bwd_ctc: the fused CTC head needs the whole-sequence kernels (amdspeech_lstm_ctc_fusable)");
    prof_flops(1, 0.0, 0.0);
    return AMDSPEECH_OK;
}
static BwdArgs bwd_args(const BwdCall& c) {
    const amdspeech_lstm_desc* d = c.d;
    float* ws = c.ws;
    const LstmLayout& lo = c.lo;
    BwdArgs a;
    a.hoist = 0; a.l0 = 0; a.mt0 = 0;
    a.wq = ws + lo.wq; a.cs = ws + lo.cs; a.gates = ws + lo.gates; a.dg = ws + lo.dg;
    a.dztop = ws + lo.dztop; a.dc = ws + lo.dc; a.lengths = c.lengths; a.dgp = ws + lo.dgp;
    a.T = d->T; a.B = d->B; a.H = d->H; a.L = d->L; a.drop = drop_cfg(d);
    return a;
}
static int weight_grads(hipStream_t s, const BwdCall& c, int ta, int tb, int dz_tb) {
    const amdspeech_lstm_desc* d = c.d;
    const LstmLayout& lo = c.lo;
    float* ws = c.ws;
    const int T = d->T, B = d->B, H = d->H, L = d->L;
    const size_t TB = (size_t)T * B, r0 = (size_t)ta * B;
    const int rows = (tb - ta) * B, dz_rows = (dz_tb - ta) * B;
    for (int l = 0; l < L; ++l) {
        const float* z = ws + lo.z + ((size_t)l * TB + r0) * H;
        const float* hp = ws + lo.hs + ((size_t)l * (T + 1) * B + r0) * H;
        const float* dg = ws + lo.dg + ((size_t)l * TB + r0) * 4 * H;
        float* dk = c.dkernels + l * c.kstride;
        float* db = c.dbiases + l * c.bstride;
        if (c.p.bf16p && rows % 64 == 0 && rows >= 64) {
            if (int rc = bf16p_dk(s, bf16p_bufs(d, ws + lo.bfs), rows, H, z, hp, dg, dk, db)) return rc;
        } else if (d->precision != 0) {
            if (int rc = gemm_reduced(d, s, true, false, H, 4 * H, rows, z, H, dg, 4 * H, dk, 4 * H, nullptr, true)) return rc;
            if (int rc = colsum_accumulate(s, dg, rows, 4 * H, 4 * H, db)) return rc;
            if (int rc = gemm_reduced(d, s, true, false, H, 4 * H, rows, hp, H, dg, 4 * H, dk + (size_t)H * 4 * H, 4 * H, nullptr, true)) return rc;
        } else {
            const float* pa[2] = {z, hp}; const float* pb[2] = {dg, dg};
            float* pc[2] = {dk, dk + (size_t)H * 4 * H}; float* ps[2] = {db, nullptr};
            if (gemm_f32_tn_group_ok(H, 4 * H, rows, z, H, dg, 4 * H) && gemm_f32_tn_group_ok(H, 4 * H, rows, hp, H, dg, 4 * H)) {
                if (int rc = gemm_f32_tn_group(s, 2, H, 4 * H, rows, pa, H, pb, 4 * H, pc, 4 * H, ps, true)) return rc;
            } else {
                for (int i = 0; i < 2; ++i)
                    if (int rc = gemm_f32(s, true, false, H, 4 * H, rows, pa[i], H, pb[i], 4 * H, pc[i], 4 * H, nullptr, true, ps[i])) return rc;
            }
        }
    }
    if (dz_rows <= 0) return AMDSPEECH_OK;
    const float* dg0 = ws + lo.dg + r0 * 4 * H;
    float* dz0 = ws + lo.dz0 + r0 * H;
    if (c.p.bf16p && dz_rows >= 256) return bf16p_dx(s, bf16p_bufs(d, ws + lo.bfs), dz_rows, H, dg0, c.kernels, dz0);
    return gemm_batched(d, s, false, true, dz_rows, H, 4 * H, dg0, 4 * H, c.kernels, 4 * H, dz0, H, nullptr, false);
}
static int hand_down(hipStream_t s, const BwdCall& c, int l) {
    const amdspeech_lstm_desc* d = c.d;
    const int H = d->H;
    const size_t TB = (size_t)d->T * d->B;
    return gemm_batched(d, s, false, true, (int)TB, H, 4 * H, c.ws + c.lo.dg + (size_t)l * TB * 4 * H, 4 * H, c.kernels + l * c.kstride,
                        4 * H, c.ws + c.lo.dztop, H, nullptr, false);
}

static int bwd_flow(hipStream_t s, const BwdCall& c) {
    const amdspeech_lstm_desc* d = c.d;
    const LstmPlan& p = c.p;
    const LstmLayout& lo = c.lo;
    float* ws = c.ws;
    const int T = d->T, B = d->B, H = d->H, L = d->L;
    unsigned* err = reinterpret_cast<unsigned*>(ws + lo.sync);
    int* progress = reinterpret_cast<int*>(err) + 8;
    unsigned* tickets = err + 16;
    if (!(d->flags & AMDSPEECH_LSTM_ARMED))
        if (int rc = flow_fill_bwd_panels(s, d, ws, lo, c.head != nullptr)) return rc;
    AS_CHECK_HIP(hipMemsetD32Async(reinterpret_cast<hipDeviceptr_t>(progress), T, 8, s));
    AS_CHECK_HIP(hipMemsetAsync(tickets, 0, 16 * sizeof(unsigned), s));
#if FLOW2_CHECK_ORDER
    AS_CHECK_HIP(hipMemsetD32Async(reinterpret_cast<hipDeviceptr_t>(ws + lo.dg), (int)FLOW_SENTINEL, (size_t)L * T * B * 4 * H, s));
    AS_CHECK_HIP(hipMemsetAsync(ws + lo.pdown, 0, (lo.total - lo.pdown) * sizeof(float), s));
#endif
    FlowBwdArgs fb;
    fb.wq = ws + lo.wq; fb.cs = ws + lo.cs; fb.gates = ws + lo.gates; fb.dg = ws + lo.dg; fb.dztop = ws + lo.dztop;
    fb.prec = ws + lo.prec; fb.pdown = ws + lo.pdown;
    fb.nprog = p.nmt; fb.prog_slack = 0;
    fb.dxh = ws + lo.dxh; fb.tickets = tickets; fb.lengths = c.lengths; fb.err = err; fb.progress = progress;
    fb.T = T; fb.B = B; fb.H = H; fb.L = L; fb.drop = drop_cfg(d);
    fb.limit = p.limit;
    fb.trace = dev_trace_ptr();
    fb.trace_layer = dev_knob("AMDSPEECH_TRACE_LAYER", L - 1);
    fb.cf = CtcFlow{}; fb.cf_on = 0;
    if (c.head != nullptr) {
        AS_CHECK_ARG(p.nfw > 0, "lstm_bwd_ctc: this shape does not take the fused CTC head (amdspeech_lstm_ctc_fusable)");
        fb.cf = ctc_head_args(d, c.head, ws, lo, nullptr, p.nfw); fb.cf_on = 1;
        fb.cf.lengths = c.lengths; fb.cf.err = err; fb.cf.limit = fb.limit;
    }
    AS_CHECK_HIP(hipFuncSetAttribute(reinterpret_cast<const void*>(p.bwd_flow), hipFuncAttributeMaxDynamicSharedMemorySize, (int)p.bwd_lds));
    fb.z = ws + lo.z; fb.hs = ws + lo.hs; fb.kernels = c.kernels; fb.dk = c.dkernels; fb.dbias = c.dbiases; fb.dz0 = ws + lo.dz0;
    fb.kstride = c.kstride; fb.bstride = c.bstride;
    fb.dz0_inkernel = p.dz0_inkernel;
    fb.w_dz0 = p.w_dz0;
    fb.w_mode = 0;
    fb.w_pieces = p.w_pieces;
    fb.w_counters = p.w_deal ? tickets + 8 : nullptr;
    fb.w_t0 = p.w_t0;
    prof_begin(1, s);
    hipLaunchKernelGGL(p.bwd_flow, dim3(256), dim3(512), p.bwd_lds, s, fb);
    prof_end(1, s, T + L - 1);
    if (int rc = flow_mark_postlaunch(s, ws, 1 | (fb.dz0_inkernel ? 2 : 0))) return rc;
    {
        const double prod = 2.0 * B * 4 * H * H;
        const double wframes = fb.w_pieces > 0 ? (double)(T - fb.w_t0) : 0.0;
        prof_flops(1, (double)T * (2 * L - 1 + (fb.dz0_inkernel ? 1 : 0)) * prod,
                   wframes * (L * 2.0 * prod + (fb.w_dz0 ? prod : 0.0)));
    }
    AS_CHECK_LAUNCH();
    if (int rc = weight_grads(s, c, 0, p.w_pieces > 0 ? p.w_t0 : T, p.dz0_inkernel ? 0 : T)) return rc;
    return p.dz0_inkernel ? AMDSPEECH_OK : mask_dz0(s, c);
}

static int big1_bwd_layers(hipStream_t s, int n, const BwdCall* st) {
    const amdspeech_lstm_desc* d = st[0].d;
    const int T = d->T, B = d->B, H = d->H, L = d->L, nmt = ceil_div(B, 16);
    const size_t TB = (size_t)T * B;
    const size_t pring_floats = (size_t)2 * nmt * 2 * 32 * 32 * 256, xring_floats = (size_t)2 * nmt * 64 * 1024;
    BigBwd1Args b1;
    b1.n = n;
    for (int k = 0; k < n; ++k) {
        const BwdCall& q = st[k];
        const LstmLayout& lo = q.lo;
        unsigned* err = reinterpret_cast<unsigned*>(q.ws + lo.sync);
        BigBwdArgs& b2 = b1.b[k];
        b2.wq = q.ws + lo.wq; b2.cs = q.ws + lo.cs; b2.gates = q.ws + lo.gates; b2.dg = q.ws + lo.dg; b2.dup = q.ws + lo.dztop;
        b2.lengths = q.lengths; b2.pring = q.ws + lo.bigring; b2.xring = q.ws + lo.bigring + pring_floats; b2.err = err; b2.tickets = err + 16;
        b2.T = T; b2.B = B; b2.H = H; b2.L = L; b2.drop = drop_cfg(q.d);
        b2.limit = q.p.limit;
    }
    for (int l = L - 1; l >= 0; --l) {
        for (int k = 0; k < n; ++k) {
            AS_CHECK_HIP(hipMemsetAsync(b1.b[k].pring, 0, (pring_floats + xring_floats) * sizeof(float), s));
            AS_CHECK_HIP(hipMemsetAsync(b1.b[k].tickets, 0, 8 * sizeof(unsigned), s));
            b1.b[k].layer = l;
            const Bf16pBufs bufs = bf16p_bufs(st[k].d, st[k].ws + st[k].lo.bfs);
            b1.b[k].dgb = bufs.dgb; b1.b[k].dbias = st[k].dbiases + l * st[k].bstride;
        }
        if (n == 1) b1.b[1] = b1.b[0];
        prof_begin(1, s, L - 1 - l);
        hipLaunchKernelGGL(lstm_bwd_big1<BIG1_Q>, dim3(256), dim3(512), 0, s, b1);
        prof_end(1, s, T * L, L - 1 - l);
        for (int k = 0; k < n; ++k) {
            const BwdCall& q = st[k];
            float* ws = q.ws;
            if (int rc = bf16p_layer_bwd_copied(s, bf16p_bufs(q.d, ws + q.lo.bfs), (int)TB, H, ws + q.lo.z + (size_t)l * TB * H,
                                                ws + q.lo.hs + (size_t)l * (T + 1) * B * H, q.kernels + l * q.kstride,
                                                l > 0 ? ws + q.lo.dztop : ws + q.lo.dz0, q.dkernels + l * q.kstride)) return rc;
        }
    }
    AS_CHECK_LAUNCH();
    for (int k = 0; k < n; ++k)
        if (int rc = mask_dz0(s, st[k])) return rc;
// ... 192 lines not shown
__global__ void export_zmult_kernel(float* out, long n, DropCfg c, int lp) {
    long i = (long)blockIdx.x * blockDim.x + threadIdx.x;
    if (i < n) out[i] = zmult(c, lp, (uint32_t)i);
}
extern "C" int amdspeech_lstm_dropout_multipliers(void* stream, const amdspeech_lstm_desc* d, int which, int layer, float* out) {
    if (int rc = check_desc(d)) return rc;
    AS_CHECK_ARG(out != nullptr && (which == 0 || which == 1) && layer >= 0 && layer < d->L,
                 "lstm_dropout_multipliers: which must be 0 (input mask) or 1 (output mask), layer in [0, L)");
    DropCfg dc{which == 0 ? d->keep_in : 1.0f, which == 1 ? d->keep_out : 1.0f, d->seed, d->L};
    const long n = (long)d->T * d->B * d->H;
    hipLaunchKernelGGL(export_zmult_kernel, dim3(ceil_div(n, 256)), dim3(256), 0, static_cast<hipStream_t>(stream), out, n, dc,
                       which == 0 ? layer : layer + 1);
    AS_CHECK_LAUNCH();
    return AMDSPEECH_OK;
}

extern "C" int amdspeech_lstm_workspace_release(void* stream, void* ws) {
    AS_CHECK_ARG(ws != nullptr, "lstm_workspace_release: null workspace");
    return flow_arm_release(static_cast<hipStream_t>(stream), ws);
}

extern "C" int amdspeech_lstm_beside_forward(void* stream, const void* ws) {
    AS_CHECK_ARG(ws != nullptr, "lstm_beside_forward: null workspace");
    std::lock_guard<std::mutex> lock(g_arm_mutex);
    auto it = g_arm.find(ws);
    if (it == g_arm.end() || it->second.idle_xcds <= 0 || it->second.pre == nullptr) return 0;
    AS_CHECK_HIP(hipStreamWaitEvent(static_cast<hipStream_t>(stream), it->second.pre, 0));
    return it->second.idle_xcds;
}

extern "C" int amdspeech_lstm_beside_tail(void* stream, const void* ws) {
    AS_CHECK_ARG(ws != nullptr, "lstm_beside_tail: null workspace");
    std::lock_guard<std::mutex> lock(g_arm_mutex);
    auto it = g_arm.find(ws);
    if (it == g_arm.end() || it->second.post_flags == 0 || it->second.post == nullptr) return 0;
    AS_CHECK_HIP(hipStreamWaitEvent(static_cast<hipStream_t>(stream), it->second.post, 0));
    return it->second.post_flags;
}

extern "C" int amdspeech_lstm_status(const amdspeech_lstm_desc* d, void* ws) {
    if (int rc = check_desc(d)) return rc;
    AS_CHECK_ARG(ws != nullptr, "lstm_status: null workspace");
    const LstmLayout lo = lstm_layout(lstm_plan(d, nullptr));
    unsigned err = 0;
    AS_CHECK_HIP(hipMemcpy(&err, static_cast<float*>(ws) + lo.sync, sizeof(err), hipMemcpyDeviceToHost));
    if (err != 0) {
        flow_xw_forget(ws);
        set_error("LSTM dataflow kernels: a bounded wait timed out (flags 0x%x: 1 = forward, 2 = backward -- the workgroups of "
                  "one launch were not all resident; 4 = a weight-gradient GEMM gave up waiting for the backward kernel, "
                  "8 = an x-product worker of the forward kernel gave up waiting for the layer below, "
                  "32 = the fused CTC head gave up waiting for the top layer, "
                  "e.g. under a tool that serialises kernels: set AMDSPEECH_FLOW_GEMM=0:0); results of this step are invalid", err);
        return AMDSPEECH_ETIMEOUT;
    }
    return AMDSPEECH_OK;
}

extern "C" int amdspeech_lstm_fwd(void* stream, const amdspeech_lstm_desc* d, void* ws, const float* kernels,
                                  long kernel_stride, const float* biases, long bias_stride,
                                  const int* lengths, const float* h0, const float* c0) {
    return lstm_fwd(static_cast<hipStream_t>(stream), FwdCall{d, static_cast<float*>(ws), kernels, kernel_stride, biases, bias_stride, lengths, h0, c0});
}

extern "C" int amdspeech_lstm_pair_fusable(const amdspeech_lstm_desc* d) {
    return d != nullptr && check_desc(d) == AMDSPEECH_OK && lstm_plan(d, nullptr).pair;
}
static bool pair_together(const amdspeech_lstm_desc* d_a, const void* ws_a, const amdspeech_lstm_desc* d_b, const void* ws_b) {
    return d_a->T == d_b->T && d_a->B == d_b->B && d_a->H == d_b->H && d_a->L == d_b->L && d_a->precision == d_b->precision &&
           ws_a != ws_b && amdspeech_lstm_pair_fusable(d_a) && amdspeech_lstm_pair_fusable(d_b);
}

extern "C" int amdspeech_lstm_fwd_pair(void* stream, const amdspeech_lstm_desc* d_a, void* ws_a, const float* kernels_a, const float* biases_a,
                                       const amdspeech_lstm_desc* d_b, void* ws_b, const float* kernels_b, const float* biases_b,
                                       long kernel_stride, long bias_stride, const int* lengths, const float* h0_a, const float* c0_a) {
    hipStream_t s = static_cast<hipStream_t>(stream);
    AS_CHECK_ARG(d_a && d_b, "lstm_fwd_pair: null descriptor");
    FwdCall two[2] = {{d_a, static_cast<float*>(ws_a), kernels_a, kernel_stride, biases_a, bias_stride, lengths, h0_a, c0_a},
                      {d_b, static_cast<float*>(ws_b), kernels_b, kernel_stride, biases_b, bias_stride, lengths, nullptr, nullptr}};
    if (!pair_together(d_a, ws_a, d_b, ws_b)) {
        if (int rc = lstm_fwd(s, two[0])) return rc;
        return lstm_fwd(s, two[1]);
    }
    for (FwdCall& c : two) {
        if (int rc = fwd_prologue(s, c)) return rc;
        if (int rc = fwd_stage(s, c)) return rc;
    }
    return big_fwd_layers(s, 2, two, true);
}

extern "C" int amdspeech_lstm_bwd_pair(void* stream, const amdspeech_lstm_desc* d_a, void* ws_a, const float* kernels_a, float* dkernels_a,
                                       float* dbiases_a, const amdspeech_lstm_desc* d_b, void* ws_b, const float* kernels_b, float* dkernels_b,
                                       float* dbiases_b, long kernel_stride, long bias_stride, const int* lengths) {
    hipStream_t s = static_cast<hipStream_t>(stream);
    AS_CHECK_ARG(d_a && d_b, "lstm_bwd_pair: null descriptor");
    BwdCall two[2] = {{d_a, static_cast<float*>(ws_a), kernels_a, kernel_stride, dkernels_a, dbiases_a, bias_stride, lengths},
                      {d_b, static_cast<float*>(ws_b), kernels_b, kernel_stride, dkernels_b, dbiases_b, bias_stride, lengths}};
    if (!pair_together(d_a, ws_a, d_b, ws_b) || lstm_plan(d_a, nullptr).bwd != Path::big1) {
        if (int rc = lstm_bwd(s, two[0])) return rc;
        return lstm_bwd(s, two[1]);
    }
    for (BwdCall& c : two)
        if (int rc = bwd_prologue(s, c)) return rc;
    return big1_bwd_layers(s, 2, two);
}

extern "C" int amdspeech_lstm_bwd(void* stream, const amdspeech_lstm_desc* d, void* ws, const float* kernels,
                                  long kernel_stride, float* dkernels, float* dbiases, long bias_stride,
                                  const int* lengths) {
    return lstm_bwd(static_cast<hipStream_t>(stream), BwdCall{d, static_cast<float*>(ws), kernels, kernel_stride, dkernels, dbiases, bias_stride, lengths});
}

extern "C" int amdspeech_lstm_plan(const amdspeech_lstm_desc* d, int C, int U, amdspeech_lstm_plan_info* out) {
    if (int rc = check_desc(d)) return rc;
    AS_CHECK_ARG(out != nullptr, "lstm_plan: null output");
    AS_CHECK_ARG((C > 0 && U > 0) || (C == 0 && U == 0), "lstm_plan: head C=%d U=%d (both 0: no head)", C, U);
    amdspeech_ctc_head h{};
    h.C = C; h.U = U;
    const LstmPlan p = lstm_plan(d, C > 0 ? &h : nullptr);
    const bool flow_bwd = p.bwd == Path::flow;
    static_assert((int)Path::flow == AMDSPEECH_LSTM_PATH_FLOW && (int)Path::big1 == AMDSPEECH_LSTM_PATH_BIG1 &&
                  (int)Path::big == AMDSPEECH_LSTM_PATH_BIG && (int)Path::hoist == AMDSPEECH_LSTM_PATH_HOIST &&
                  (int)Path::diag == AMDSPEECH_LSTM_PATH_DIAG && (int)Path::diag_bf3 == AMDSPEECH_LSTM_PATH_DIAG_BF3, "amdspeech.h");
    *out = amdspeech_lstm_plan_info{(int)p.fwd, (int)p.bwd, p.nmt, p.fwd == Path::flow ? d->H / 128 : 0, p.mv, p.wpx, p.uw, p.fwd_mt,
                                    p.pair ? 1 : 0, p.bf16p ? 1 : 0, p.bf16p_reserved ? 1 : 0, p.xw_parts, p.nfw, p.w_pieces,
                                    p.dz0_inkernel, flow_bwd ? flow2_q(d->H / 128, d->precision) : 0};
    return AMDSPEECH_OK;
}
extern "C" int amdspeech_lstm_plan_xw_halves(const amdspeech_lstm_desc* d, int C, int U) {
    if (check_desc(d) != AMDSPEECH_OK) return -1;
    amdspeech_ctc_head h{};
    h.C = C; h.U = U;
    const LstmPlan p = lstm_plan(d, C > 0 ? &h : nullptr);
    return 2 * p.mv + p.mh;
}
extern "C" int amdspeech_lstm_plan_xw_ksteps(const amdspeech_lstm_desc* d, int C, int U) {
    if (check_desc(d) != AMDSPEECH_OK) return -1;
    amdspeech_ctc_head h{};
    h.C = C; h.U = U;
    const LstmPlan p = lstm_plan(d, C > 0 ? &h : nullptr);
    return p.me;
}
extern "C" int amdspeech_lstm_ctc_fusable(const amdspeech_lstm_desc* d, int C, int U) {
    if (check_desc(d) != AMDSPEECH_OK) return 0;
    amdspeech_ctc_head h{};
    h.C = C; h.U = U;
    return lstm_plan(d, &h).nfw > 0 ? 1 : 0;
}
static int check_head(const amdspeech_ctc_head* h, bool bwd) {
    AS_CHECK_ARG(h != nullptr, "lstm_*_ctc: null head");
    AS_CHECK_ARG(h->w_out && h->b_out && h->logits && h->dense_labels && h->loss && h->ctc_ws && (!bwd || h->dlogits),
                 "lstm_*_ctc: null pointer in the head");
    AS_CHECK_ARG(((uintptr_t)h->w_out % 16) == 0 && ((uintptr_t)h->ctc_ws % 256) == 0, "lstm_*_ctc: W_o must be 16-byte, the CTC workspace 256-byte aligned");
    return AMDSPEECH_OK;
}
extern "C" int amdspeech_lstm_fwd_ctc(void* stream, const amdspeech_lstm_desc* d, void* ws, const float* kernels,
                                      long kernel_stride, const float* biases, long bias_stride, const int* lengths,
                                      const float* h0, const float* c0, const amdspeech_ctc_head* head) {
    if (int rc = check_head(head, false)) return rc;
    return lstm_fwd(static_cast<hipStream_t>(stream), FwdCall{d, static_cast<float*>(ws), kernels, kernel_stride, biases, bias_stride, lengths, h0, c0, head});
}
extern "C" int amdspeech_lstm_bwd_ctc(void* stream, const amdspeech_lstm_desc* d, void* ws, const float* kernels,
                                      long kernel_stride, float* dkernels, float* dbiases, long bias_stride,
                                      const int* lengths, const amdspeech_ctc_head* head) {
    if (int rc = check_head(head, true)) return rc;
    return lstm_bwd(static_cast<hipStream_t>(stream), BwdCall{d, static_cast<float*>(ws), kernels, kernel_stride, dkernels, dbiases, bias_stride, lengths, head});
}

namespace amdspeech {
#include "lstm_layer.h"
#include "lstm_layer_bf3.h"
#include "lstm_bidir.h"
}
```

### rnn-speech_amd/engine.py

```python
import contextlib
import math
import os

import numpy as np
import torch

from . import lib as _lib
from . import ops


def _pad64(n):
    return (n + 63) // 64 * 64


class ParamLayout(object):

    def __init__(self, num_layers, hidden, input_dim, num_labels, bidirectional=False, bidirectional_mode="top"):
        self.L, self.H, self.D, self.C = num_layers, hidden, input_dim, num_labels
        self.bidirectional = bool(bidirectional)
        self.layerwise = self.bidirectional and bidirectional_mode == "layer"
        off = 0
        self.slots = {}

        def take(name, shape):
            nonlocal off
            n = 1
            for s in shape:
                n *= s
            self.slots[name] = (off, shape)
            off += _pad64(n)

        take("input_w", (input_dim, hidden))
        take("input_b", (hidden,))
        def rows(l):
            return (3 if self.layerwise and l > 0 else 2) * hidden

        for l in range(num_layers):
            take("kernel_%d" % l, (rows(l), 4 * hidden))
            take("bias_%d" % l, (4 * hidden,))
        if self.bidirectional:
            for l in range(num_layers):
                take("bw_kernel_%d" % l, (rows(l), 4 * hidden))
                take("bw_bias_%d" % l, (4 * hidden,))
        take("output_w", ((2 if self.bidirectional else 1) * hidden, num_labels))
        take("output_b", (num_labels,))
        self.total = off
        if self.layerwise:
            self.kernel_stride = self.bias_stride = None
        elif num_layers > 1:
            self.kernel_stride = self.slots["kernel_1"][0] - self.slots["kernel_0"][0]
            self.bias_stride = self.slots["bias_1"][0] - self.slots["bias_0"][0]
        else:
            self.kernel_stride = self.bias_stride = 0

    def names(self):
        return list(self.slots.keys())

    def view(self, flat, name):
        off, shape = self.slots[name]
        n = 1
        for s in shape:
            n *= s
        return flat[off:off + n].view(*shape)

    def num_params(self):
        tot = 0
        for _, shape in self.slots.values():
            n = 1
            for s in shape:
                n *= s
            tot += n
        return tot


_BESIDE_FORWARD = os.environ.get("AMDSPEECH_BESIDE_FORWARD", "1") != "0"
_BESIDE_TAIL = os.environ.get("AMDSPEECH_BESIDE_TAIL", "1") != "0"
_BIDIR_PAIR = os.environ.get("AMDSPEECH_BIDIR_PAIR", "1") != "0"
_FUSED_CTC = os.environ.get("AMDSPEECH_FUSED_CTC", "1") != "0"


PRECISIONS = {"f32": 0, "bf16x3": 1, "bf16": 2}


class ParamStore(object):

    def __init__(self, layout, device):
        self.layout, self.device = layout, torch.device(device)
        self.params, self.grads, self.adam_m, self.adam_v = (torch.zeros(layout.total, device=self.device) for _ in range(4))
        self.norm = torch.zeros(1, device=self.device)
        self.adam_step = 0

    def p(self, name):
        return self.layout.view(self.params, name)

    def g(self, name):
        return self.layout.view(self.grads, name)

    def init_parameters(self, seed=1234):
        gen = torch.Generator(device="cpu")
        gen.manual_seed(seed)
        self.params.zero_()
        for name in self.layout.names():
            _, shape = self.layout.slots[name]
            if len(shape) == 2:
                lim = math.sqrt(6.0 / (shape[0] + shape[1]))
                w = (torch.rand(shape, generator=gen) * 2.0 - 1.0) * lim
                self.p(name).copy_(w)

    def load_numpy(self, arrays, flat=None):
        flat = self.params if flat is None else flat
        for name, a in arrays.items():
            if name not in self.layout.slots:
                raise KeyError("unknown parameter tensor %r (layout has %s)" % (name, ", ".join(self.layout.names())))
            want = tuple(self.layout.slots[name][1])
            got = tuple(np.shape(a))
            if got != want:
                raise ValueError("checkpoint tensor %s has shape %s, %s needs %s" % (name, got, self._describe(), want))
            self.layout.view(flat, name).copy_(torch.as_tensor(np.asarray(a), dtype=torch.float32))

    def to_numpy(self, flat=None):
        flat = self.params if flat is None else flat
        return {n: self.layout.view(flat, n).detach().cpu().numpy().copy() for n in self.layout.names()}

    def zero_grads(self):
        self.grads.zero_()

    def apply(self, lr, clip, beta1=0.9, beta2=0.999, eps=1e-8):
        self.adam_step += 1
        t = self.adam_step
        lr_t = lr * math.sqrt(1.0 - beta2 ** t) / (1.0 - beta1 ** t)
        ops.clip_adam(self.params, self.grads, self.adam_m, self.adam_v, float(clip), lr_t, beta1, beta2, eps,
                      norm_out=self.norm)
        return self.norm

    def healthy(self):
        try:
            self.check()
            return True
        except _lib.DataflowTimeout:
            return False

    def _run_length(self, max_len):
        return self.T if max_len is None else max(1, min(int(max_len), self.T))


class Engine(ParamStore):
    def __init__(self, num_layers, hidden, input_dim, num_labels, batch_size, max_T, max_U,
                 device="cuda", seed=1234, normalization=False, precision="f32", bidirectional=False,
                 sync_batch_norm=False, bidirectional_mode="top"):
        if not torch.cuda.is_available():
            raise RuntimeError("rnn_speech_amd needs a ROCm GPU (MI355X); there is no CPU path")
        self.L, self.H, self.D, self.C = num_layers, hidden, input_dim, num_labels
        self.B, self.T, self.U = batch_size, max_T, max_U
        self.bidirectional = bool(bidirectional)
        if bidirectional_mode not in ("top", "layer"):
            raise ValueError("bidirectional_mode must be 'top' (two stacks joined in front of the output layer) or 'layer' "
                             "(stack_bidirectional_dynamic_rnn: every layer reads both directions of the layer below)")
        self.layerwise = self.bidirectional and bidirectional_mode == "layer"
        if self.layerwise and precision not in ("f32", "bf16x3"):
            raise ValueError("bidirectional_mode 'layer' runs in exact f32 or bf16x3 (precision %r requested): the layer-wise kernels "
                             "have no plain-bf16 variant" % (precision,))
        ParamStore.__init__(self, ParamLayout(num_layers, hidden, input_dim, num_labels, bidirectional=self.bidirectional,
                                              bidirectional_mode="layer" if self.layerwise else "top"), device)
        if precision not in PRECISIONS:
            raise ValueError("precision must be 'f32' (exact, default), 'bf16x3' (split-precision MFMA) or 'bf16' (plain bf16 "
                             "operands, f32 accumulation and master weights)")
        self.precision = precision
        if self.layerwise:
            self.lstm_ws = ops.BidirWorkspace(max_T, batch_size, hidden, num_layers, device=self.device, precision=PRECISIONS[precision])
        else:
            self.lstm_ws = ops.LstmWorkspace(max_T, batch_size, hidden, num_layers, device=self.device, precision=PRECISIONS[precision])
        if self.bidirectional and not self.layerwise:
            self.lstm_ws_b = ops.LstmWorkspace(max_T, batch_size, hidden, num_layers, device=self.device,
                                               precision=PRECISIONS[precision])
            self.ytop_b = torch.empty(max_T, batch_size, hidden, device=self.device)
            self.dytop_b = torch.empty(max_T, batch_size, hidden, device=self.device)
        self.ctc_ws = ops.CtcWorkspace(max_T, batch_size, num_labels, max_U, self.device)
        self.logits = torch.empty(max_T, batch_size, num_labels, device=self.device)
        self.dlogits = torch.empty_like(self.logits)
        self.loss = torch.zeros(batch_size, device=self.device)
        self.state_h = torch.zeros(num_layers, batch_size, hidden, device=self.device)
        self.state_c = torch.zeros(num_layers, batch_size, hidden, device=self.device)
        self.normalization = bool(normalization)
        self.sync_batch_norm = bool(sync_batch_norm) and self.normalization
        if self.normalization:
            self.bn_xhat = torch.empty(max_T, batch_size, hidden, device=self.device)
            self.bn_inv_std = torch.empty(max_T, hidden, device=self.device)
            self.bn_scratch = torch.empty(2, max_T, hidden, device=self.device)
        self._ws, self._Tr = self.lstm_ws, max_T
        self._head = None
        self._per_diagonal = False
        self._paired = False
        self._ws_b = self.lstm_ws_b if self.bidirectional and not self.layerwise else None
        self.stream = torch.cuda.Stream(device=self.device, priority=-1)
        self._aux_stream = None
        self._tail_stream = None
        self.init_parameters(seed)

    def _describe(self):
        return "the model (L=%d, H=%d, D=%d, C=%d)" % (self.L, self.H, self.D, self.C)

    @staticmethod
    def _dp_group():
        from . import dataparallel
        return dataparallel.current()

    def _run_length(self, max_len):
        if max_len is not None and self.sync_batch_norm and self._dp_group().world > 1:
            return self.T
        return ParamStore._run_length(self, max_len)

    def forward(self, x, lengths, keep_in=1.0, keep_out=1.0, seed=0, use_state=False, max_len=None, after_lstm=None, training=False,
                per_diagonal=False, dense_labels=None):
        T, B, D = x.shape
        assert (T, B, D) == (self.T, self.B, self.D), ((T, B, D), (self.T, self.B, self.D))
        x = x.contiguous()
        Tr = self._run_length(max_len)
        ws = self.lstm_ws.prefix(Tr)
        self._ws, self._Tr = ws, Tr
        ws.set_dropout(keep_in, keep_out, seed)
        ops.linear_fwd(x[:Tr].view(Tr * B, D), self.p("input_w"), self.p("input_b"), out=ws.z0.view(Tr * B, self.H))
        if self.normalization:
            grp = self._dp_group() if self.sync_batch_norm else None
            if grp is not None and grp.world > 1:
                ops.batchnorm_fwd_dp(ws.z0, ws.z0, self.bn_xhat, self.bn_inv_std, grp, self.bn_scratch, 1e-3)
            else:
                ops.batchnorm_fwd(ws.z0, ws.z0, self.bn_xhat[:Tr], self.bn_inv_std[:Tr], 1e-3)
        if self.layerwise:
            return self._forward_layerwise(ws, lengths, keep_in, keep_out, seed, use_state, after_lstm, per_diagonal, Tr)
        if self.bidirectional:
            wb = self.lstm_ws_b.prefix(Tr)
            self._ws_b = wb
            ops.reverse_sequences(ws.z0, lengths, out=wb.z0)
        self._per_diagonal = bool(per_diagonal)
        self._head = None
        if (dense_labels is not None and _FUSED_CTC and not self.bidirectional
                and ops.lstm_ctc_fusable(ws, self.C, dense_labels.shape[1], per_diagonal=per_diagonal)):
            self._head = ops.CtcHead(self.p("output_w"), self.p("output_b"), self.logits[:Tr], dense_labels, self.loss,
                                     self.dlogits[:Tr], self.ctc_ws)
        paired = self.bidirectional and _BIDIR_PAIR and not per_diagonal and ops.lstm_pair_fusable(ws)
        self._paired = bool(paired)
        if paired:
            wb.set_dropout(keep_in, keep_out, seed ^ 0x5bd1e995)
            ops.lstm_fwd_pair(ws, self.p("kernel_0"), self.p("bias_0"), wb, self.p("bw_kernel_0"), self.p("bw_bias_0"),
                              self.layout.kernel_stride, self.layout.bias_stride, lengths,
                              self.state_h if use_state else None, self.state_c if use_state else None)
        else:
            ops.lstm_fwd(ws, self.p("kernel_0"), self.layout.kernel_stride, self.p("bias_0"),
                         self.layout.bias_stride, lengths,
                         self.state_h if use_state else None, self.state_c if use_state else None, training=training,
                         per_diagonal=per_diagonal, head=self._head)
        H = self.H
        if not self.bidirectional:
            if after_lstm is not None:
                after_lstm()
            if self._head is None:
                ops.linear_fwd(ws.ztop.view(Tr * B, H), self.p("output_w"), self.p("output_b"),
                               out=self.logits[:Tr].view(Tr * B, self.C))
        else:
            if not paired:
                wb.set_dropout(keep_in, keep_out, seed ^ 0x5bd1e995)
                ops.lstm_fwd(wb, self.p("bw_kernel_0"), self.layout.kernel_stride, self.p("bw_bias_0"),
                             self.layout.bias_stride, lengths, None, None, training=training, per_diagonal=per_diagonal)
            if after_lstm is not None:
                after_lstm()
            ops.reverse_sequences(wb.ztop, lengths, out=self.ytop_b[:Tr])
            wo = self.p("output_w")
            ops.linear_fwd(ws.ztop.view(Tr * B, H), wo[:H], self.p("output_b"), out=self.logits[:Tr].view(Tr * B, self.C))
            ops.gemm(self.ytop_b[:Tr].view(Tr * B, H), wo[H:], out=self.logits[:Tr].view(Tr * B, self.C), accumulate=True)
        if Tr < T:
            self.logits[Tr:] = self.p("output_b")
        return self.logits

    def _cells(self, flat):
        L = self.L
        ks = [self.layout.view(flat, "kernel_%d" % l) for l in range(L)] + [self.layout.view(flat, "bw_kernel_%d" % l) for l in range(L)]
        bs = [self.layout.view(flat, "bias_%d" % l) for l in range(L)] + [self.layout.view(flat, "bw_bias_%d" % l) for l in range(L)]
        return ks, bs

    def _forward_layerwise(self, ws, lengths, keep_in, keep_out, seed, use_state, after_lstm, per_diagonal, Tr):
        B, H = self.B, self.H
        ws.set_dropout(keep_in, keep_out, seed)
        ks, bs = self._cells(self.params)
        self._per_diagonal = bool(per_diagonal)
        ops.lstm_bidir_fwd(ws, ks, bs, lengths, self.state_h if use_state else None, self.state_c if use_state else None,
                           per_frame=per_diagonal)
        if after_lstm is not None:
            after_lstm()
        wo = self.p("output_w")
        ops.linear_fwd(ws.ytop_fw.view(Tr * B, H), wo[:H], self.p("output_b"), out=self.logits[:Tr].view(Tr * B, self.C))
        ops.gemm(ws.ytop_bw.view(Tr * B, H), wo[H:], out=self.logits[:Tr].view(Tr * B, self.C), accumulate=True)
        if Tr < self.T:
            self.logits[Tr:] = self.p("output_b")
        return self.logits

    def kernel_path(self):
        path = {"fused_ctc_head": self._head is not None, "paired": self._paired, "run_length": self._Tr}
        if not self.layerwise:
            plan = ops.lstm_plan(self._ws, head=self._head, per_diagonal=self._per_diagonal)
            path["lstm_fwd"], path["lstm_bwd"] = ("big1" if self._paired else plan["fwd_path"]), plan["bwd_path"]
        if self.layerwise:
            plan = ops.lstm_bidir_plan(self._ws, per_frame=self._per_diagonal)
            path["layer_recurrence"] = {2: "persistent", 1: "persistent_per_direction", 0: "per_frame"}[plan["path"]]
            path["layer_product"] = self.precision
        return path

    def final_state(self):
        return self._ws.final_state()

    def keep_state(self):
        h, c = self._ws.final_state()
        self.state_h.copy_(h)
        self.state_c.copy_(c)

    def zero_state(self):
        self.state_h.zero_()
        self.state_c.zero_()

    def ctc(self, dense_labels, lengths, stage=0):
        Tr = self._Tr
        if self._head is not None:
            if Tr < self.T and stage != 1:
                self.dlogits[Tr:].zero_()
            return self.loss
        ops.ctc_loss_fwd_bwd(self.logits[:Tr], dense_labels, lengths, ws=self.ctc_ws, loss=self.loss,
                             dlogits=self.dlogits[:Tr], stage=stage)
        if Tr < self.T and stage != 1:
            self.dlogits[Tr:].zero_()
        return self.loss

    def align(self, x, lengths, dense_labels):
        self.forward(x, lengths)
        shape = (self.T, self.B, self.C, dense_labels.shape[1])
        if getattr(self, "_align_ws", None) is None or self._align_ws.shape != shape:
# ... 195 lines not shown
```

### rnn-speech_amd/lib.py

```python
import ctypes as C
import os

HERE = os.path.dirname(os.path.abspath(__file__))
LIB_PATH = os.environ.get("AMDSPEECH_LIB") or os.path.join(HERE, "libamdspeech.so")


class AmdSpeechError(RuntimeError):
    pass


class DataflowTimeout(AmdSpeechError):
    """amdspeech_lstm_status returned AMDSPEECH_ETIMEOUT: a whole-sequence launch gave up waiting.  The mini-batch's results are
    invalid; it can be repeated on the launch-per-diagonal kernels.  Any OTHER error of that call is a device fault."""


ETIMEOUT = -4
ECALLBACK = -100


class LstmDesc(C.Structure):
    _fields_ = [("T", C.c_int), ("B", C.c_int), ("H", C.c_int), ("L", C.c_int),
                ("keep_in", C.c_float), ("keep_out", C.c_float), ("seed", C.c_uint64),
                ("precision", C.c_int), ("flags", C.c_int)]


class CtcHead(C.Structure):
    _fields_ = [("w_out", C.c_void_p), ("b_out", C.c_void_p), ("logits", C.c_void_p), ("dense_labels", C.c_void_p),
                ("loss", C.c_void_p), ("dlogits", C.c_void_p), ("ctc_ws", C.c_void_p), ("C", C.c_int), ("U", C.c_int)]


class LstmPlanInfo(C.Structure):
    _fields_ = [(n, C.c_int) for n in ("fwd_path", "bwd_path", "nmt", "kb", "mv", "wpx", "uw", "fwd_mt", "pair", "bf16p", "bf16p_reserved",
                                       "xw_parts", "nfw", "w_pieces", "dz0_inkernel", "flow2_q")]


class LstmBidirPlanInfo(C.Structure):
    _fields_ = [(n, C.c_int) for n in ("path", "cus", "fwd_kpw", "fwd_waves", "fwd_groups", "fwd_wgs", "fwd_lds", "bwd_kpw", "bwd_waves",
                                       "bwd_groups", "bwd_wgs", "bwd_lds")]


class CtcPlanInfo(C.Structure):
    _fields_ = [(n, C.c_int) for n in ("kernel", "threads", "rmax", "smax")]


class GemmPlanInfo(C.Structure):
    _fields_ = [(n, C.c_int) for n in ("family", "variant", "splits", "k_chunk", "atomic", "zero_fill", "grid", "tiles_m", "tiles_n", "map",
                                       "bm", "bn", "col_slices", "a_vec", "b_vec")]


class FrontendPlanInfo(C.Structure):
    _fields_ = [(n, C.c_int) for n in ("frames_kernel", "maxq", "n_dft", "frame_len", "hop", "n_bins", "bin_tiles", "kp", "lds_bytes", "t_full",
                                       "tiles_per_utt", "n_items", "workgroups", "dct_kernel", "dct_col_tiles", "meta_by_copy")]


class FrameStackPlanInfo(C.Structure):
    _fields_ = [(n, C.c_int) for n in ("t_out", "d_out", "vec", "workgroups", "meta_by_copy")]


class SpecAugmentDesc(C.Structure):
    _fields_ = [(n, C.c_int) for n in ("period", "freq_masks", "freq_width", "time_masks", "time_width", "time_permille")] + \
               [("seed", C.c_uint64)]


class SpecAugmentPlanInfo(C.Structure):
    _fields_ = [(n, C.c_int) for n in ("vec", "lanes", "items_per_workgroup", "workgroups", "reps")]


class FeatureNormDesc(C.Structure):
    _fields_ = [("mode", C.c_int), ("norm_vars", C.c_int), ("var_floor", C.c_double)]


class FeatureNormPlanInfo(C.Structure):
    _fields_ = [(n, C.c_int) for n in ("vec", "split", "workgroups", "lds_bytes", "meta_by_copy", "workspace_bytes")]


class ResampleRowsPlanInfo(C.Structure):
    _fields_ = [(n, C.c_int) for n in ("tile", "tiles_per_row", "workgroups", "span_max", "table_chunk", "lds_bytes", "any_copy", "meta_launches")]


class ReverbRowsPlanInfo(C.Structure):
    _fields_ = [(n, C.c_int) for n in ("tile", "tiles_per_row", "workgroups", "taps", "span_max", "k_chunk", "k_chunks", "lds_bytes", "copy_rows",
                                       "meta_launches")]


class NoiseMixRowsPlanInfo(C.Structure):
    _fields_ = [(n, C.c_int) for n in ("tile", "tiles_per_row", "workgroups", "lds_bytes", "copy_rows", "meta_launches")]


class XentPlanInfo(C.Structure):
    _fields_ = [(n, C.c_int) for n in ("kernel", "values_per_lane", "threads", "rows_per_workgroup", "grid", "c_min", "c_max", "loss_threads",
                                       "loss_grid")]


class LmStepPlanInfo(C.Structure):
    _fields_ = [(n, C.c_int) for n in ("kernel", "row_tile", "threads", "launches", "n_min", "n_max", "col_tiles", "row_tiles", "lds_bytes",
                                       "out_row_tile", "out_row_tiles", "v_max")]


LM_STEP_FN = C.CFUNCTYPE(C.c_int, C.c_void_p, C.c_int, C.POINTER(C.c_int), C.POINTER(C.c_int), C.POINTER(C.c_int), C.POINTER(C.c_float))

GEMM_FAMILIES = ("skinny_n", "skinny_k", "skinny_tn", "tn_direct", "kc_direct", "lds", "bf3", "bf16p")
GEMM_MAP_LINEAR, GEMM_MAP_XCD, GEMM_MAP_XCD_BLOCKS, GEMM_MAP_KC_BAND = range(4)
GEMM_GROUP_MAX = 10
CTC_KERNELS = ("wave", "shift", "pair", "edge")
LSTM_PATHS = ("flow", "big1", "big", "hoist", "diag", "diag_bf3")
XENT_KERNELS = ("wave", "block")
LM_STEP_KERNELS = ("mfma16",)
FEATURE_NORM_MODES = ("none", "utterance", "global")
LSTM_ARMED, LSTM_ARM_NEXT, LSTM_SAME_WS, LSTM_PER_DIAGONAL, LSTM_INJECT_TIMEOUT = 1, 2, 4, 8, 16


COMM_ID_BYTES = 128
WS_Z0, WS_ZTOP, WS_DZTOP, WS_DZ0, WS_HFINAL, WS_CFINAL, WS_GATES = range(7)
BIDIR_WS_Z0, BIDIR_WS_YTOP_FW, BIDIR_WS_YTOP_BW, BIDIR_WS_DYTOP_FW, BIDIR_WS_DYTOP_BW, BIDIR_WS_DZ0, BIDIR_WS_HFINAL, BIDIR_WS_CFINAL = range(8)

_P = C.c_void_p
_I = C.c_int
_F = C.c_float
_L = C.c_long
_SZ = C.c_size_t

PROTOTYPES = {
    "amdspeech_version": (_I, []),
    "amdspeech_last_error": (C.c_char_p, []),
    "amdspeech_device_cu_count": (_I, []),
    "amdspeech_linear_fwd": (_I, [_P, _P, _P, _P, _P, _I, _I, _I]),
    "amdspeech_linear_bwd": (_I, [_P, _P, _P, _P, _P, _P, _P, _I, _I, _I]),
    "amdspeech_gemm_f32": (_I, [_P, _I, _I, _I, _I, _I, _P, _I, _P, _I, _P, _I, _P, _I]),
    "amdspeech_gemm_bf16x3": (_I, [_P, _I, _I, _I, _I, _I, _P, _I, _P, _I, _P, _I, _P, _I]),
    "amdspeech_gemm_bf16": (_I, [_P, _I, _I, _I, _I, _I, _P, _I, _P, _I, _P, _I, _P, _I]),
    "amdspeech_gemm_plan": (_I, [_I, _I, _I, _I, _I, _I, _P, _I, _P, _I, _P, _I, _P, _I, _I, _I, C.POINTER(GemmPlanInfo)]),
    "amdspeech_gemm_f32_tn_group": (_I, [_P, _I, _I, _I, _I, _P, _I, _P, _I, _P, _I, _P, _I]),
    "amdspeech_colsum_accumulate": (_I, [_P, _P, _I, _I, _I, _P]),
    "amdspeech_gemm_bf16_packed_scratch_bytes": (_SZ, [_I, _I, _I, _I, _I, _I, _I]),
    "amdspeech_gemm_bf16_packed": (_I, [_P, _I, _I, _I, _I, _I, _P, _I, _P, _I, _P, _I, _P, _I, _P, _SZ]),
    "amdspeech_gemm_bf16_packed_plan": (_I, [_I, _I, _I, _I, _I, _I, _I, C.POINTER(GemmPlanInfo)]),
    "amdspeech_bf16_copy": (_I, [_P, _P, C.c_long, C.c_long, _I, _I, _P, C.c_long, _P, _P]),
    "amdspeech_bf16_transpose": (_I, [_P, _P, C.c_long, _I, _P, C.c_long]),
    "amdspeech_batchnorm_fwd": (_I, [_P, _P, _P, _P, _P, _I, _I, _I, _F]),
    "amdspeech_batchnorm_bwd": (_I, [_P, _P, _P, _P, _P, _I, _I, _I]),
    "amdspeech_batchnorm_sum": (_I, [_P, _P, _P, _I, _P, _I, _I, _I]),
    "amdspeech_batchnorm_apply": (_I, [_P, _P, _P, _P, _I, _F, _P, _P, _P, _I, _I, _I]),
    "amdspeech_batchnorm_bwd_sums": (_I, [_P, _P, _P, _P, _I, _I, _I]),
    "amdspeech_batchnorm_bwd_apply": (_I, [_P, _P, _P, _P, _P, _I, _P, _I, _I, _I]),
    "amdspeech_lstm_workspace_bytes": (_SZ, [C.POINTER(LstmDesc)]),
    "amdspeech_lstm_ws_ptr": (_P, [C.POINTER(LstmDesc), _P, _I]),
    "amdspeech_lstm_fwd": (_I, [_P, C.POINTER(LstmDesc), _P, _P, _L, _P, _L, _P, _P, _P]),
    "amdspeech_lstm_status": (_I, [C.POINTER(LstmDesc), _P]),
    "amdspeech_lstm_workspace_release": (_I, [_P, _P]),
    "amdspeech_lstm_beside_forward": (_I, [_P, _P]),
    "amdspeech_lstm_beside_tail": (_I, [_P, _P]),
    "amdspeech_lstm_bwd": (_I, [_P, C.POINTER(LstmDesc), _P, _P, _L, _P, _P, _L, _P]),
    "amdspeech_lstm_ctc_fusable": (_I, [C.POINTER(LstmDesc), _I, _I]),
    "amdspeech_lstm_pair_fusable": (_I, [C.POINTER(LstmDesc)]),
    "amdspeech_lstm_fwd_pair": (_I, [_P, C.POINTER(LstmDesc), _P, _P, _P, C.POINTER(LstmDesc), _P, _P, _P, _L, _L, _P, _P, _P]),
    "amdspeech_lstm_bwd_pair": (_I, [_P, C.POINTER(LstmDesc), _P, _P, _P, _P, C.POINTER(LstmDesc), _P, _P, _P, _P, _L, _L, _P]),
    "amdspeech_lstm_fwd_ctc": (_I, [_P, C.POINTER(LstmDesc), _P, _P, _L, _P, _L, _P, _P, _P, C.POINTER(CtcHead)]),
    "amdspeech_lstm_bwd_ctc": (_I, [_P, C.POINTER(LstmDesc), _P, _P, _L, _P, _P, _L, _P, C.POINTER(CtcHead)]),
    "amdspeech_lstm_dropout_multipliers": (_I, [_P, C.POINTER(LstmDesc), _I, _I, _P]),
    "amdspeech_lstm_plan": (_I, [C.POINTER(LstmDesc), _I, _I, C.POINTER(LstmPlanInfo)]),
    "amdspeech_lstm_plan_xw_halves": (_I, [C.POINTER(LstmDesc), _I, _I]),
    "amdspeech_lstm_plan_xw_ksteps": (_I, [C.POINTER(LstmDesc), _I, _I]),
    "amdspeech_lstm_bidir_workspace_bytes": (_SZ, [C.POINTER(LstmDesc)]),
    "amdspeech_lstm_bidir_ws_ptr": (_P, [C.POINTER(LstmDesc), _P, _I]),
    "amdspeech_lstm_bidir_layer_stride": (_L, [C.POINTER(LstmDesc)]),
    "amdspeech_lstm_bidir_path": (_I, [C.POINTER(LstmDesc)]),
    "amdspeech_lstm_bidir_plan": (_I, [C.POINTER(LstmDesc), C.POINTER(LstmBidirPlanInfo)]),
    "amdspeech_lstm_bidir_fwd": (_I, [_P, C.POINTER(LstmDesc), _P, _P, _P, _P, _P, _P]),
    "amdspeech_lstm_bidir_bwd": (_I, [_P, C.POINTER(LstmDesc), _P, _P, _P, _P, _P]),
    "amdspeech_lstm_bidir_status": (_I, [C.POINTER(LstmDesc), _P]),
    "amdspeech_lstm_bidir_dropout_multipliers": (_I, [_P, C.POINTER(LstmDesc), _I, _I, _I, _P]),
    "amdspeech_ctc_workspace_bytes": (_SZ, [_I, _I, _I, _I]),
    "amdspeech_ctc_plan": (_I, [_I, _I, _I, _I, C.POINTER(CtcPlanInfo)]),
    "amdspeech_ctc_loss_fwd_bwd": (_I, [_P, _P, _P, _P, _I, _I, _I, _I, _P, _P, _P]),
    "amdspeech_ctc_loss_fwd_bwd_staged": (_I, [_P, _P, _P, _P, _I, _I, _I, _I, _P, _P, _P, _I]),
    "amdspeech_ctc_align_workspace_bytes": (_SZ, [_I, _I, _I, _I]),
    "amdspeech_ctc_align_plan": (_I, [_I, _I, _I, _I, C.POINTER(CtcPlanInfo)]),
    "amdspeech_ctc_align": (_I, [_P, _P, _P, _P, _I, _I, _I, _I, _P, _P, _P, _P, _P, _P]),
    "amdspeech_ctc_greedy_decode": (_I, [_P, _P, _P, _I, _I, _I, _P, _P, _P]),
    "amdspeech_merge_repeated": (_I, [_P, _P, _P, _I, _I, _I]),
    "amdspeech_edit_distance": (_I, [_P, _P, _P, _I, _P, _P, _I, _I, _P]),
    "amdspeech_ctc_beam_search_host": (_I, [_P, _P, _I, _I, _I, _I, _I, _P, _P, _P]),
    "amdspeech_ctc_beam_search_host_mt": (_I, [_P, _P, _I, _I, _I, _I, _I, _P, _P, _P, _I]),
    "amdspeech_ctc_beam_search_host_nbest": (_I, [_P, _P, _I, _I, _I, _I, _I, _I, _P, _P, _P, _P, _I]),
    "amdspeech_edit_distance_host": (_I, [_P, _P, _I, _P, _P, _I, _I, _P]),
    "amdspeech_crc32c": (C.c_uint32, [_P, _SZ, C.c_uint32]),
    "amdspeech_resample_workspace_bytes": (_SZ, [C.c_int]),
    "amdspeech_resample_num_samples": (C.c_int, [C.c_int, C.c_int, C.c_int]),
    "amdspeech_resample": (C.c_int, [_P, _P, C.POINTER(C.c_int), C.c_int, C.c_int, C.c_int, C.c_int, _P, C.c_int, _P]),
    "amdspeech_resample_rows_num_samples": (C.c_int, [C.c_int, C.c_int, C.c_int, C.c_int]),
    "amdspeech_resample_rows_workspace_bytes": (_SZ, [C.c_int]),
    "amdspeech_resample_rows": (C.c_int, [_P, _P, C.POINTER(C.c_int), C.POINTER(C.c_int), C.c_int, C.c_int, C.c_int, C.c_int, _P, C.c_int, _P]),
    "amdspeech_resample_rows_plan": (C.c_int, [C.POINTER(C.c_int), C.POINTER(C.c_int), C.c_int, C.c_int, C.c_int, C.c_int, C.c_int,
                                               C.POINTER(ResampleRowsPlanInfo)]),
    "amdspeech_speed_perturb_draw": (C.c_int, [C.c_uint64, C.c_uint64, C.POINTER(C.c_int), C.c_int]),
    "amdspeech_reverb_rows_workspace_bytes": (_SZ, [_I]),
    "amdspeech_reverb_rows": (_I, [_P, _P, C.POINTER(_I), _I, _I, _P, C.POINTER(_I), C.POINTER(_I), _I, _I, C.POINTER(_I), _P, _P]),
    "amdspeech_reverb_rows_plan": (_I, [C.POINTER(_I), _I, _I, C.POINTER(_I), C.POINTER(_I), _I, _I, C.POINTER(_I),
                                        C.POINTER(ReverbRowsPlanInfo)]),
    "amdspeech_row_sumsq_workspace_bytes": (_SZ, [_I]),
    "amdspeech_row_sumsq": (_I, [_P, _P, C.POINTER(_I), _I, _I, _P, _P]),
    "amdspeech_noise_mix_rows_workspace_bytes": (_SZ, [_I]),
    "amdspeech_noise_mix_rows": (_I, [_P, _P, C.POINTER(_I), _I, _I, _P, C.POINTER(_I), _P, _I, _I, _P, C.POINTER(_I), C.POINTER(_I),
                                      C.POINTER(_I), _P, _P]),
    "amdspeech_noise_mix_rows_plan": (_I, [C.POINTER(_I), _I, _I, C.POINTER(_I), _I, _I, C.POINTER(_I), C.POINTER(_I), C.POINTER(_I),
                                           C.POINTER(NoiseMixRowsPlanInfo)]),
    "amdspeech_augment_draw": (_I, [C.c_uint64, C.c_uint64, _I, _I, _I, _I, C.POINTER(_I), _I, _I, C.POINTER(_I)]),
    "amdspeech_audio_probe": (C.c_int, [C.c_char_p, C.POINTER(C.c_int), C.POINTER(C.c_int), C.POINTER(C.c_long)]),
    "amdspeech_audio_decode": (C.c_int, [C.c_char_p, _P, C.c_long, C.POINTER(C.c_long), C.POINTER(C.c_int), C.c_int]),
    "amdspeech_optim_workspace_bytes": (_SZ, [_L]),
    "amdspeech_clip_adam": (_I, [_P, _P, _P, _P, _P, _L, _F, _F, _F, _F, _F, _P, _P]),
    "amdspeech_frontend_workspace_bytes": (_SZ, [_I, _I, _I, _I]),
    "amdspeech_frontend_num_frames": (_I, [_I, _I, _I]),
    "amdspeech_frontend_plan": (_I, [_I, _I, _I, _I, _I, _I, C.POINTER(FrontendPlanInfo)]),
    "amdspeech_frontend_mfcc": (_I, [_P, _P, _P, _I, _I, _I, _I, _I, _P, _P, _P]),
    "amdspeech_frontend_fbank": (_I, [_P, _P, _P, _I, _I, _I, _I, _P, _P, _P]),
    "amdspeech_frame_stack_num_frames": (_I, [_I, _I]),
    "amdspeech_frame_stack": (_I, [_P, _P, _P, _I, _I, _I, _I, _I, _P, _P]),
    "amdspeech_frame_stack_plan": (_I, [_I, _I, _I, _I, _I, C.POINTER(FrameStackPlanInfo)]),
    "amdspeech_spec_augment": (_I, [_P, _P, _P, _I, _I, _I, C.POINTER(SpecAugmentDesc)]),
    "amdspeech_spec_augment_spans": (_I, [C.POINTER(SpecAugmentDesc), _I, _I, C.POINTER(C.c_int)]),
    "amdspeech_spec_augment_plan": (_I, [_I, _I, _I, C.POINTER(SpecAugmentDesc), C.POINTER(SpecAugmentPlanInfo)]),
    "amdspeech_feature_norm_plan": (_I, [_I, _I, _I, _I, C.POINTER(FeatureNormPlanInfo)]),
    "amdspeech_feature_moments": (_I, [_P, _P, _P, _I, _I, _I, _P, _P]),
    "amdspeech_feature_norm": (_I, [_P, _P, _P, _I, _I, _I, C.POINTER(FeatureNormDesc), _P, _P]),
    "amdspeech_profile_enable": (_I, [_I]),
    "amdspeech_profile_get": (_I, [_I, C.POINTER(C.c_float), C.POINTER(C.c_int)]),
    "amdspeech_profile_get_flops": (_I, [_I, C.POINTER(C.c_double), C.POINTER(C.c_double)]),
    "amdspeech_comm_available": (_I, []),
    "amdspeech_comm_unique_id": (_I, [_P]),
    "amdspeech_comm_init": (_I, [_P, _I, _I, C.POINTER(_P)]),
    "amdspeech_comm_destroy": (_I, [_P]),
    "amdspeech_comm_info": (_I, [_P, C.POINTER(_I), C.POINTER(_I), C.POINTER(_I), C.c_char_p, _I]),
    "amdspeech_allreduce_sum_f32": (_I, [_P, _P, _P, _L]),
    "amdspeech_broadcast_f32": (_I, [_P, _P, _P, _L, _I]),
    "amdspeech_reverse_sequences": (_I, [_P, _P, _P, _P, _I, _I, _I, _I]),
    "amdspeech_axpy": (_I, [_P, _F, _P, _P, _L]),
    "amdspeech_fill": (_I, [_P, _P, _F, _L]),
    "amdspeech_embed_fwd": (_I, [_P, _P, _I, _P, _I, _I, _I, _I, _P, _P, _P]),
    "amdspeech_embed_bwd_workspace_bytes": (_SZ, [_I, _I, _I, _I]),
    "amdspeech_embed_bwd": (_I, [_P, _P, _I, _P, _I, _I, _I, _I, _P, _P, _P, _P]),
# ... 35 lines not shown
```

### rnn-speech_amd/ops.py

```python
import ctypes as C
import os

import torch

from . import lib as _l

MODE_MFCC, MODE_FBANK = 0, 1


def _stream():
    return C.c_void_p(torch.cuda.current_stream().cuda_stream)


def _p(t):
    return C.c_void_p(t.data_ptr()) if t is not None else C.c_void_p(0)


def _chk_f32(*ts):
    for t in ts:
        if t is None:
            continue
        if not (t.is_cuda and t.dtype == torch.float32 and t.is_contiguous()):
            raise ValueError("expected a contiguous float32 device tensor, got %s %s" % (t.dtype, t.device))

# ... 294 lines not shown
    _TOO_SMALL = "lstm workspace: the layout for T = %d needs %d bytes, the shared allocation has %d"

    def __init__(self, T, B, H, L, keep_in=1.0, keep_out=1.0, seed=0, device="cuda", precision=0, _share=None):
        _StackWorkspace.__init__(self, T, B, H, L, keep_in, keep_out, seed, device, precision, _share)
        self.z0 = self._view(_l.WS_Z0, (T, B, H))
        self.ztop = self._view(_l.WS_ZTOP, (T, B, H))
        self.dztop = self._view(_l.WS_DZTOP, (T, B, H))
        self.dz0 = self._view(_l.WS_DZ0, (T, B, H))
        self._armed = None
        self._ever_armed = False
        self._fwd_seen = False
        self._lib_state = False

    def __del__(self):
        try:
            if self._root is self and (self._ever_armed or self._fwd_seen or self._lib_state) and torch.cuda.is_available():
                self.lib.amdspeech_lstm_workspace_release(_stream(), _p(self.buf))
        except Exception:
            pass

    def final_state(self):
        T, B, H, L = self.T, self.B, self.H, self.L
        stride = (T + 1) * B * H
        oh, oc = self._offset(_l.WS_HFINAL), self._offset(_l.WS_CFINAL)
        h = torch.as_strided(self.buf, (L, B, H), (stride, H, 1), oh)
        c = torch.as_strided(self.buf, (L, B, H), (stride, H, 1), oc)
        return h, c


_ARM = os.environ.get("AMDSPEECH_ARM", "1") != "0"


class CtcHead(object):

    def __init__(self, w_out, b_out, logits, dense_labels, loss, dlogits, ctc_ws):
        _chk_f32(w_out, b_out, logits, loss, dlogits)
        _chk_i32(dense_labels)
        T, B, C_ = logits.shape
        if ctc_ws.shape[0] < T or tuple(ctc_ws.shape[1:]) != (B, C_, dense_labels.shape[1]):
            raise ValueError("CtcHead: the CTC workspace was sized for %r, the logits are %r with U = %d"
                             % (ctc_ws.shape, (T, B, C_), dense_labels.shape[1]))
        self.keep = (w_out, b_out, logits, dense_labels, loss, dlogits, ctc_ws)
        self.c = _l.CtcHead(_p(w_out).value, _p(b_out).value, _p(logits).value, _p(dense_labels).value, _p(loss).value,
                            _p(dlogits).value if dlogits is not None else None, _p(ctc_ws.buf).value, C_, dense_labels.shape[1])


def lstm_ctc_fusable(ws, C_, U, per_diagonal=False):
    if per_diagonal:
        return False
    return bool(ws.lib.amdspeech_lstm_ctc_fusable(C.byref(ws.desc), int(C_), int(U)))


def lstm_plan(ws, head=None, per_diagonal=False):
    c_u = (0, 0) if head is None else ((head.c.C, head.c.U) if isinstance(head, CtcHead) else (int(head[0]), int(head[1])))
    d = _l.LstmDesc(ws.desc.T, ws.desc.B, ws.desc.H, ws.desc.L, ws.desc.keep_in, ws.desc.keep_out, ws.desc.seed, ws.desc.precision,
                    _l.LSTM_PER_DIAGONAL if per_diagonal else 0)
    info = _l.LstmPlanInfo()
    _l.check(ws.lib.amdspeech_lstm_plan(C.byref(d), c_u[0], c_u[1], C.byref(info)), "lstm_plan")
    out = _plan_dict(info)
    out["fwd_path"], out["bwd_path"] = _l.LSTM_PATHS[out["fwd_path"]], _l.LSTM_PATHS[out["bwd_path"]]
    return out


def lstm_plan_xw_halves(ws, head=None, per_diagonal=False):
    c_u = (0, 0) if head is None else ((head.c.C, head.c.U) if isinstance(head, CtcHead) else (int(head[0]), int(head[1])))
    d = _l.LstmDesc(ws.desc.T, ws.desc.B, ws.desc.H, ws.desc.L, ws.desc.keep_in, ws.desc.keep_out, ws.desc.seed, ws.desc.precision,
                    _l.LSTM_PER_DIAGONAL if per_diagonal else 0)
    n = int(ws.lib.amdspeech_lstm_plan_xw_halves(C.byref(d), c_u[0], c_u[1]))
    if n < 0:
        raise ValueError("lstm_plan_xw_halves: bad descriptor")
    return n


def lstm_plan_xw_ksteps(ws, head=None, per_diagonal=False):
    c_u = (0, 0) if head is None else ((head.c.C, head.c.U) if isinstance(head, CtcHead) else (int(head[0]), int(head[1])))
    d = _l.LstmDesc(ws.desc.T, ws.desc.B, ws.desc.H, ws.desc.L, ws.desc.keep_in, ws.desc.keep_out, ws.desc.seed, ws.desc.precision,
                    _l.LSTM_PER_DIAGONAL if per_diagonal else 0)
    n = int(ws.lib.amdspeech_lstm_plan_xw_ksteps(C.byref(d), c_u[0], c_u[1]))
    if n < 0:
        raise ValueError("lstm_plan_xw_ksteps: bad descriptor")
    return n


def lstm_fwd(ws, kernels, kernel_stride, biases, bias_stride, lengths, h0=None, c0=None, training=False, per_diagonal=False, head=None):
    _chk_i32(lengths)
    _chk_f32(h0, c0)
    root, key = ws._root, (ws.T, int(ws.desc.precision))
    if per_diagonal:
        root._armed, training = None, False
    armed = _ARM and root._armed is not None and root._armed["fwd"] == key
    root._armed = None
    inject, root._inject_timeout = getattr(root, "_inject_timeout", 0), 0
    ws.desc.flags = ((_l.LSTM_ARMED if armed else 0) | (_l.LSTM_ARM_NEXT if (training and _ARM) else 0) |
                     (_l.LSTM_SAME_WS if (root._fwd_seen and _ARM) else 0) | (_l.LSTM_PER_DIAGONAL if per_diagonal else 0) |
                     (_l.LSTM_INJECT_TIMEOUT if inject else 0))
    root._fwd_seen = False
    try:
        if head is None:
            _l.check(ws.lib.amdspeech_lstm_fwd(_stream(), C.byref(ws.desc), _p(ws.buf), _p(kernels), kernel_stride,
                                               _p(biases), bias_stride, _p(lengths), _p(h0), _p(c0)), "lstm_fwd")
        else:
            _l.check(ws.lib.amdspeech_lstm_fwd_ctc(_stream(), C.byref(ws.desc), _p(ws.buf), _p(kernels), kernel_stride,
                                                   _p(biases), bias_stride, _p(lengths), _p(h0), _p(c0), C.byref(head.c)), "lstm_fwd_ctc")
        root._fwd_seen = not per_diagonal
        root._lib_state = True
    finally:
        ws.desc.flags = 0
    if training and _ARM:
        root._armed = {"fwd": key, "bwd": key}
        root._ever_armed = True


def lstm_pair_fusable(ws):
    ws.desc.flags = 0
    return bool(ws.lib.amdspeech_lstm_pair_fusable(C.byref(ws.desc)))


def lstm_fwd_pair(ws_a, kernels_a, biases_a, ws_b, kernels_b, biases_b, kernel_stride, bias_stride, lengths, h0=None, c0=None):
    _chk_i32(lengths)
    _chk_f32(h0, c0)
    for ws in (ws_a, ws_b):
        ws._root._armed, ws._root._fwd_seen, ws._root._lib_state = None, False, True
        ws.desc.flags = 0
    _l.check(ws_a.lib.amdspeech_lstm_fwd_pair(_stream(), C.byref(ws_a.desc), _p(ws_a.buf), _p(kernels_a), _p(biases_a),
                                              C.byref(ws_b.desc), _p(ws_b.buf), _p(kernels_b), _p(biases_b),
                                              kernel_stride, bias_stride, _p(lengths), _p(h0), _p(c0)), "lstm_fwd_pair")


def lstm_status(ws):
    try:
        _l.check(ws.lib.amdspeech_lstm_status(C.byref(ws.desc), _p(ws.buf)), "lstm_status")
    except _l.AmdSpeechError:
        ws._root._armed = None
        ws._root._fwd_seen = False
        raise


def lstm_beside_forward(ws, stream):
    rc = _l.load().amdspeech_lstm_beside_forward(C.c_void_p(stream.cuda_stream), _p(ws._root.buf))
    if rc < 0:
        _l.check(rc, "lstm_beside_forward")
    return rc


def lstm_beside_tail(ws, stream):
    rc = _l.load().amdspeech_lstm_beside_tail(C.c_void_p(stream.cuda_stream), _p(ws._root.buf))
    if rc < 0:
        _l.check(rc, "lstm_beside_tail")
    return rc


def lstm_bwd(ws, kernels, kernel_stride, dkernels, dbiases, bias_stride, lengths, per_diagonal=False, head=None):
    _chk_i32(lengths)
    root, key = ws._root, (ws.T, int(ws.desc.precision))
    armed = root._armed is not None and root._armed["bwd"] == key and not per_diagonal
    if root._armed is not None:
        root._armed["bwd"] = None
    root._lib_state = True
    inject, root._inject_timeout_bwd = getattr(root, "_inject_timeout_bwd", 0), 0
    ws.desc.flags = ((_l.LSTM_ARMED if armed else 0) | (_l.LSTM_PER_DIAGONAL if per_diagonal else 0) |
                     (_l.LSTM_INJECT_TIMEOUT if inject else 0))
    try:
        if head is None:
            _l.check(ws.lib.amdspeech_lstm_bwd(_stream(), C.byref(ws.desc), _p(ws.buf), _p(kernels), kernel_stride,
                                               _p(dkernels), _p(dbiases), bias_stride, _p(lengths)), "lstm_bwd")
        else:
            _l.check(ws.lib.amdspeech_lstm_bwd_ctc(_stream(), C.byref(ws.desc), _p(ws.buf), _p(kernels), kernel_stride,
                                                   _p(dkernels), _p(dbiases), bias_stride, _p(lengths), C.byref(head.c)), "lstm_bwd_ctc")
    finally:
        ws.desc.flags = 0


def lstm_bwd_pair(ws_a, kernels_a, dkernels_a, dbiases_a, ws_b, kernels_b, dkernels_b, dbiases_b, kernel_stride, bias_stride, lengths):
    _chk_i32(lengths)
    for ws in (ws_a, ws_b):
        if ws._root._armed is not None:
            ws._root._armed["bwd"] = None
        ws._root._lib_state = True
        ws.desc.flags = 0
    _l.check(ws_a.lib.amdspeech_lstm_bwd_pair(_stream(), C.byref(ws_a.desc), _p(ws_a.buf), _p(kernels_a), _p(dkernels_a), _p(dbiases_a),
                                              C.byref(ws_b.desc), _p(ws_b.buf), _p(kernels_b), _p(dkernels_b), _p(dbiases_b),
# ... 718 lines not shown
```

Before: 2.747 million.

## Fuse input projection with dropout mask and packed staging into skinny GEMM

Moves the input linear layer into the LSTM forward call. When the flow path applies, the skinny-K GEMM epilogue applies the dropout multipliers and writes the packed per-frame layout directly, so the separate mask_pack_rows pass over z is skipped. It also pre-arms the backward progress and ticket sync words in the forward prepare kernel on a separate region, with a dedicated backward join event, so backward avoids its memsets. This adds epilogue work and extra stores in the GEMM, and makes the armed sync state more complex.

```diff
diff --git a/include/amdspeech.h b/include/amdspeech.h
--- a/include/amdspeech.h
+++ b/include/amdspeech.h
@@ -135,6 +135,18 @@
 int amdspeech_lstm_bwd_ctc(void* stream, const amdspeech_lstm_desc* d, void* ws,
                            const float* kernels, long kernel_stride, float* dkernels, float* dbiases, long bias_stride,
                            const int* lengths, const amdspeech_ctc_head* head);
+
+typedef struct amdspeech_lstm_input {
+    const float* x;
+    const float* w;
+    const float* b;
+    int D;
+} amdspeech_lstm_input;
+int amdspeech_lstm_fwd_in(void* stream, const amdspeech_lstm_desc* d, void* ws,
+                          const float* kernels, long kernel_stride, const float* biases, long bias_stride,
+                          const int* lengths, const float* h0, const float* c0, const amdspeech_ctc_head* head,
+                          const amdspeech_lstm_input* in);
+int amdspeech_lstm_input_plan(const amdspeech_lstm_desc* d, int C, int U, void* ws, const amdspeech_lstm_input* in);
 
 int amdspeech_lstm_dropout_multipliers(void* stream, const amdspeech_lstm_desc* d, int which, int layer, float* out);
 
diff --git a/rnn-speech_amd/csrc/common.h b/rnn-speech_amd/csrc/common.h
--- a/rnn-speech_amd/csrc/common.h
+++ b/rnn-speech_amd/csrc/common.h
@@ -126,4 +126,22 @@
     return b >> 8;
 }
 
+struct DropCfg { float keep_in, keep_out; uint64_t seed; int L; };
+
+__device__ __forceinline__ float zmult(const DropCfg& c, int lp, uint32_t idx) {
+    float m = 1.0f;
+    if (c.keep_in < 1.0f && lp < c.L)
+        m *= (uniform01(c.seed, 2u * lp, idx) < c.keep_in) ? (1.0f / c.keep_in) : 0.0f;
+    if (c.keep_out < 1.0f && lp >= 1)
+        m *= (uniform01(c.seed, 2u * (lp - 1) + 1u, idx) < c.keep_out) ? (1.0f / c.keep_out) : 0.0f;
+    return m;
 }
+__device__ __forceinline__ size_t packed_off(int row, int k, int K) {
+    return ((((size_t)(row >> 4) * (K >> 4) + (k >> 4)) * 64) + (((k >> 2) & 3) * 16 + (row & 15))) * 4 + (k & 3);
+}
+
+bool gemm_skinny_stage_ok(int M, int N, int K, const float* x, const float* w, const float* bias, const float* z, int frame_rows);
+int gemm_skinny_stage_launch(hipStream_t s, int M, int N, int K, const float* x, const float* w, const float* bias, float* z, float* xp0,
+                             int frame_rows, const DropCfg& drop);
+
+}
diff --git a/rnn-speech_amd/csrc/gemm_skinny.hip b/rnn-speech_amd/csrc/gemm_skinny.hip
--- a/rnn-speech_amd/csrc/gemm_skinny.hip
+++ b/rnn-speech_amd/csrc/gemm_skinny.hip
@@ -9,6 +9,9 @@
 struct SkinnyArgs {
     const float* A; const float* B; float* C; const float* bias;
     int M, N, K, lda, ldb, ldc, accumulate;
+};
+struct SkinnyStage {
+    float* xp0; int frame_rows; DropCfg drop;
 };
 
 constexpr unsigned SK_OOB = 0x80000000u;
@@ -131,8 +134,8 @@
     for (int nt = 0; nt < NT; ++nt) out.store(off[nt], acc[nt] + add[nt]);
 }
 
-template <int KT, bool B_KC>
-__global__ __launch_bounds__(256) void gemm_skinny_k_kernel(SkinnyArgs g) {
+template <int KT, bool B_KC, bool STAGE = false>
+__global__ __launch_bounds__(256) void gemm_skinny_k_kernel(SkinnyArgs g, SkinnyStage st) {
     const int tid = threadIdx.x, w = tid >> 6, lane = tid & 63, m = lane & 15, kg = lane >> 4;
     const int row0 = blockIdx.x * 128 + w * 32;
     const sk_rsrc_t ra = __builtin_amdgcn_make_buffer_rsrc(const_cast<float*>(g.A), 0, (unsigned)(((size_t)(g.M - 1) * g.lda + g.K) * 4), 0x00020000);
@@ -140,6 +143,18 @@
     const sk_rsrc_t rb = __builtin_amdgcn_make_buffer_rsrc(const_cast<float*>(g.B), 0, (unsigned)(b_extent * 4), 0x00020000);
     SkinnyOut out;
     out.init(g);
+    sk_rsrc_t rp = out.c;
+    unsigned p_row[2] = {0u, 0u}, e_row[2] = {0u, 0u};
+    if constexpr (STAGE) {
+        const unsigned frames = (unsigned)((g.M + st.frame_rows - 1) / st.frame_rows), bp = (unsigned)(st.frame_rows + 15) / 16 * 16;
+        rp = __builtin_amdgcn_make_buffer_rsrc(st.xp0, 0, frames * bp * (unsigned)g.N * 4u, 0x00020000);
+#pragma unroll
+        for (int mt = 0; mt < 2; ++mt) {
+            const int row = row0 + mt * 16 + m, t = row / st.frame_rows, b = row - t * st.frame_rows;
+            p_row[mt] = (unsigned)t * bp * (unsigned)g.N + (unsigned)packed_off(b, 0, g.N);
+            e_row[mt] = (unsigned)row * (unsigned)g.N;
+        }
+    }
 
     f32x4 a[2][KT];
 #pragma unroll
@@ -196,6 +211,22 @@
 #pragma unroll
                     for (int q = 0; q < 2; ++q)
                         acc[mt][q] = __builtin_amdgcn_mfma_f32_16x16x4f32(cur.b[q][kt][j], a[mt][kt][j], acc[mt][q], 0, 0, 0);
+        if constexpr (STAGE) {
+#pragma unroll
+            for (int mt = 0; mt < 2; ++mt)
+#pragma unroll
+                for (int q = 0; q < 2; ++q) {
+                    const unsigned n = (unsigned)((nt + q) * 16 + 4 * kg), e = e_row[mt] + n;
+                    f32x4 v = acc[mt][q];
+                    v.x *= zmult(st.drop, 0, e); v.y *= zmult(st.drop, 0, e + 1u);
+                    v.z *= zmult(st.drop, 0, e + 2u); v.w *= zmult(st.drop, 0, e + 3u);
+                    acc[mt][q] = v;
+                    const unsigned po = cur.off[mt][q] == SK_OOB ? SK_OOB : (p_row[mt] + (unsigned)(nt + q) * 256u + (unsigned)kg * 64u) * 4u;
+                    sk_u32x4 w4;
+                    w4.x = __float_as_uint(v.x); w4.y = __float_as_uint(v.y); w4.z = __float_as_uint(v.z); w4.w = __float_as_uint(v.w);
+                    __builtin_amdgcn_raw_buffer_store_b128(w4, rp, po, 0, 0);
+                }
+        }
 #pragma unroll
         for (int mt = 0; mt < 2; ++mt)
 #pragma unroll
@@ -545,8 +576,8 @@
         const dim3 grid(p.tiles_m, p.col_slices);
 #define SK_K(KT)                                                                                           \
         do {                                                                                               \
-            if (transB) hipLaunchKernelGGL((gemm_skinny_k_kernel<KT, true>), grid, block, 0, s, g);        \
-            else hipLaunchKernelGGL((gemm_skinny_k_kernel<KT, false>), grid, block, 0, s, g);              \
+            if (transB) hipLaunchKernelGGL((gemm_skinny_k_kernel<KT, true>), grid, block, 0, s, g, SkinnyStage{}); \
+            else hipLaunchKernelGGL((gemm_skinny_k_kernel<KT, false>), grid, block, 0, s, g, SkinnyStage{});       \
         } while (0)
         if (p.variant / 2 == 3) SK_K(3);
         else SK_K(5);
@@ -566,4 +597,29 @@
     return AMDSPEECH_OK;
 }
 
-}
+
+static bool stage_plan(int M, int N, int K, const float* x, const float* w, const float* bias, const float* z, int frame_rows, GemmPlan* p) {
+    if (frame_rows < 1 || N % 16 != 0 || !gemm_skinny_plan(false, M, N, K, x, K, w, N, z, N, bias, p)) return false;
+    if (p->family != AMDSPEECH_GEMM_SKINNY_K) return false;
+    const size_t frames = ((size_t)M + frame_rows - 1) / frame_rows, bp = ((size_t)frame_rows + 15) / 16 * 16;
+    return frames * bp * N * 4 < (size_t)SK_OOB && (size_t)M * N < (1ull << 32);
+}
+bool gemm_skinny_stage_ok(int M, int N, int K, const float* x, const float* w, const float* bias, const float* z, int frame_rows) {
+    GemmPlan p;
+    return stage_plan(M, N, K, x, w, bias, z, frame_rows, &p);
+}
+int gemm_skinny_stage_launch(hipStream_t s, int M, int N, int K, const float* x, const float* w, const float* bias, float* z, float* xp0,
+                             int frame_rows, const DropCfg& drop) {
+    GemmPlan p;
+    AS_CHECK_ARG(stage_plan(M, N, K, x, w, bias, z, frame_rows, &p), "input stage: the short-K kernel does not take %d x %d x %d", M, N, K);
+    SkinnyArgs g;
+    g.A = x; g.B = w; g.C = z; g.bias = bias; g.M = M; g.N = N; g.K = K; g.lda = K; g.ldb = N; g.ldc = N; g.accumulate = 0;
+    const SkinnyStage st{xp0, frame_rows, drop};
+    const dim3 grid(p.tiles_m, p.col_slices), block(256);
+    if (p.variant / 2 == 3) hipLaunchKernelGGL((gemm_skinny_k_kernel<3, false, true>), grid, block, 0, s, g, st);
+    else hipLaunchKernelGGL((gemm_skinny_k_kernel<5, false, true>), grid, block, 0, s, g, st);
+    AS_CHECK_LAUNCH();
+    return AMDSPEECH_OK;
+}
+
+}
diff --git a/rnn-speech_amd/csrc/lstm.hip b/rnn-speech_amd/csrc/lstm.hip
--- a/rnn-speech_amd/csrc/lstm.hip
+++ b/rnn-speech_amd/csrc/lstm.hip
@@ -125,16 +125,6 @@
     return AMDSPEECH_OK;
 }
 
-struct DropCfg { float keep_in, keep_out; uint64_t seed; int L; };
-
-__device__ __forceinline__ float zmult(const DropCfg& c, int lp, uint32_t idx) {
-    float m = 1.0f;
-    if (c.keep_in < 1.0f && lp < c.L)
-        m *= (uniform01(c.seed, 2u * lp, idx) < c.keep_in) ? (1.0f / c.keep_in) : 0.0f;
-    if (c.keep_out < 1.0f && lp >= 1)
-        m *= (uniform01(c.seed, 2u * (lp - 1) + 1u, idx) < c.keep_out) ? (1.0f / c.keep_out) : 0.0f;
-    return m;
-}
 
 __global__ void apply_zmult_kernel(float* x, long n, DropCfg c, int lp) {
     long i = (long)blockIdx.x * blockDim.x + threadIdx.x;
@@ -173,9 +163,6 @@
     wq[o] = kernels[l * kstride + (long)row * 4 * H + col];
 }
 
-__device__ __forceinline__ size_t packed_off(int row, int k, int K) {
-    return ((((size_t)(row >> 4) * (K >> 4) + (k >> 4)) * 64) + (((k >> 2) & 3) * 16 + (row & 15))) * 4 + (k & 3);
-}
 
 __global__ void pack_rows_kernel(const float* __restrict__ src, size_t src_stride, float* __restrict__ dst,
                                  int B, int K, int nmat) {
@@ -208,14 +195,16 @@
     *reinterpret_cast<float4*>(dst + (size_t)t * bpk + packed_off(row, k, K)) = v;
 }
 
+constexpr int FLOW_SYNC_BWD = 40;
 __global__ __launch_bounds__(256) void flow_fwd_prepare_kernel(const float* __restrict__ h0, const float* __restrict__ c0,
                                                                float* __restrict__ hs, float* __restrict__ cs,
                                                                float* __restrict__ hph, unsigned* __restrict__ sync_words,
-                                                               int T, int B, int H, int L) {
+                                                               int T, int B, int H, int L, int arm_bwd) {
     const int bp = (B + 15) / 16 * 16;
     const size_t per = (size_t)bp * H;
     const size_t i = (size_t)blockIdx.x * blockDim.x + threadIdx.x;
-    if (i < 40) sync_words[i] = 0u;
+    if (i < FLOW_SYNC_BWD) sync_words[i] = 0u;
+    else if (arm_bwd && i < FLOW_SYNC_BWD + 24) sync_words[i] = i < FLOW_SYNC_BWD + 8 ? (unsigned)T : 0u;
     if (i >= per * L) return;
     const int l = i / per;
     const size_t r = i % per;
@@ -366,6 +355,7 @@
 }
 struct ArmState {
     hipEvent_t join = nullptr; bool pending = false;
+    hipEvent_t join_bwd = nullptr; bool pending_bwd = false;
     hipEvent_t pre = nullptr; int idle_xcds = 0;
     hipEvent_t post = nullptr; int post_flags = 0;
     int clean_set = 0;
@@ -417,12 +407,26 @@
     st.pending = true;
     return AMDSPEECH_OK;
 }
-static int flow_arm_settle(hipStream_t s, const void* ws) {
+static int flow_arm_publish_bwd(const void* ws) {
+    std::lock_guard<std::mutex> lock(g_arm_mutex);
+    ArmState& st = g_arm[ws];
+    if (!st.join_bwd) AS_CHECK_HIP(hipEventCreateWithFlags(&st.join_bwd, hipEventDisableTiming));
+    AS_CHECK_HIP(hipEventRecord(st.join_bwd, g_side));
+    st.pending_bwd = true;
+    return AMDSPEECH_OK;
+}
+static int flow_arm_settle(hipStream_t s, const void* ws, bool backward = false) {
     std::lock_guard<std::mutex> lock(g_arm_mutex);
     auto it = g_arm.find(ws);
-    if (it == g_arm.end() || !it->second.pending) return AMDSPEECH_OK;
-    AS_CHECK_HIP(hipStreamWaitEvent(s, it->second.join, 0));
-    it->second.pending = false;
+    if (it == g_arm.end()) return AMDSPEECH_OK;
+    ArmState& st = it->second;
+    if (backward) {
+        if (st.pending_bwd) AS_CHECK_HIP(hipStreamWaitEvent(s, st.join_bwd, 0));
+        st.pending_bwd = false;
+        return AMDSPEECH_OK;
+    }
+    if (st.pending) AS_CHECK_HIP(hipStreamWaitEvent(s, st.join, 0));
+    st.pending = st.pending_bwd = false;
     return AMDSPEECH_OK;
 }
 static int flow_arm_release(hipStream_t s, const void* ws) {
@@ -431,6 +435,7 @@
     if (it == g_arm.end()) return AMDSPEECH_OK;
     if (it->second.pending) AS_CHECK_HIP(hipStreamWaitEvent(s, it->second.join, 0));
     if (it->second.join) (void)hipEventDestroy(it->second.join);
+    if (it->second.join_bwd) (void)hipEventDestroy(it->second.join_bwd);
     if (it->second.pre) (void)hipEventDestroy(it->second.pre);
     if (it->second.post) (void)hipEventDestroy(it->second.post);
     g_arm.erase(it);
@@ -645,7 +650,9 @@
 struct FwdCall {
     const amdspeech_lstm_desc* d; float* ws; const float* kernels; long kstride; const float* biases; long bstride;
     const int* lengths; const float* h0; const float* c0; const amdspeech_ctc_head* head;
+    const amdspeech_lstm_input* in;
     LstmPlan p; LstmLayout lo;
+    bool staged;
 };
 struct BwdCall {
     const amdspeech_lstm_desc* d; float* ws; const float* kernels; long kstride; float* dkernels; float* dbiases; long bstride;
@@ -722,6 +729,27 @@
     return AMDSPEECH_OK;
 }
 
+static bool fwd_input_fused(const FwdCall& c) {
+    const amdspeech_lstm_desc* d = c.d;
+    return c.p.fwd == Path::flow &&
+           gemm_skinny_stage_ok(d->T * d->B, d->H, c.in->D, c.in->x, c.in->w, c.in->b, c.ws + c.lo.z, d->B);
+}
+static int check_input(const amdspeech_lstm_desc* d, const amdspeech_lstm_input* in) {
+    AS_CHECK_ARG(in != nullptr && in->x && in->w && in->b && in->D > 0, "lstm_fwd_in: null pointer or D = %d in the input block", in ? in->D : 0);
+    AS_CHECK_ARG((size_t)d->T * d->B < (1ull << 31), "lstm_fwd_in: T * B too large");
+    return AMDSPEECH_OK;
+}
+static int fwd_input(hipStream_t s, FwdCall& c) {
+    c.staged = false;
+    if (c.in == nullptr) return AMDSPEECH_OK;
+    const amdspeech_lstm_desc* d = c.d;
+    if (int rc = check_input(d, c.in)) return rc;
+    float* z = c.ws + c.lo.z;
+    if (!fwd_input_fused(c)) return gemm_f32(s, false, false, d->T * d->B, d->H, c.in->D, c.in->x, c.in->D, c.in->w, d->H, z, d->H, c.in->b, false);
+    c.staged = true;
+    return gemm_skinny_stage_launch(s, d->T * d->B, d->H, c.in->D, c.in->x, c.in->w, c.in->b, z, c.ws + c.lo.xp0, d->B, drop_cfg(d));
+}
+
 static int fwd_flow(hipStream_t s, const FwdCall& c) {
     const amdspeech_lstm_desc* d = c.d;
     const LstmPlan& p = c.p;
@@ -736,9 +764,10 @@
         if (int rc = flow_fill_fwd_panels(s, d, ws, lo, set)) return rc;
     float* const panels = ws + (size_t)set * lo.fwd_set;
     hipLaunchKernelGGL(flow_fwd_prepare_kernel, dim3(ceil_div((long)L * bph, 256)), dim3(256), 0, s, c.h0, c.c0, ws + lo.hs, ws + lo.cs,
-                       panels + lo.hph, err, T, B, H, L);
-    hipLaunchKernelGGL(mask_pack_rows_kernel, dim3(ceil_div((long)T * bh / 4, 256)), dim3(256), 0, s, ws + lo.z, ws + lo.xp0, B, H, T,
-                       dc, d->keep_in < 1.0f ? 1 : 0);
+                       panels + lo.hph, err, T, B, H, L, (d->flags & AMDSPEECH_LSTM_ARM_NEXT) ? 1 : 0);
+    if (!c.staged)
+        hipLaunchKernelGGL(mask_pack_rows_kernel, dim3(ceil_div((long)T * bh / 4, 256)), dim3(256), 0, s, ws + lo.z, ws + lo.xp0, B, H, T,
+                           dc, d->keep_in < 1.0f ? 1 : 0);
     AS_CHECK_LAUNCH();
     FlowArgs fa;
     fa.wp = ws + lo.wp; fa.bias = c.biases; fa.bias_stride = c.bstride;
@@ -779,6 +808,7 @@
         const long wtotal = (long)L * 2 * H * 4 * H;
         hipLaunchKernelGGL(pack_bwd_kernel, dim3(ceil_div(wtotal, 256)), dim3(256), 0, g_side, c.kernels, c.kstride, ws + lo.wq, H, L);
         AS_CHECK_LAUNCH();
+        if (int rc = flow_arm_publish_bwd(ws)) return rc;
         if (int rc = flow_fill_fwd_panels(g_side, d, ws, lo, 1 - set)) return rc;
         if (int rc = flow_arm_publish(ws, 1 - set)) return rc;
     }
@@ -864,6 +894,7 @@
 
 static int lstm_fwd(hipStream_t s, FwdCall c) {
     if (int rc = fwd_prologue(s, c)) return rc;
+    if (int rc = fwd_input(s, c)) return rc;
     switch (c.p.fwd) {
         case Path::flow: return fwd_flow(s, c);
         case Path::big: case Path::big1: return fwd_big(s, c);
@@ -875,7 +906,7 @@
     const amdspeech_lstm_desc* d = c.d;
     if (int rc = check_desc(d)) return rc;
     AS_CHECK_ARG(c.ws && c.kernels && c.dkernels && c.dbiases && c.lengths, "lstm_bwd: null pointer");
-    if (int rc = flow_arm_settle(s, c.ws)) return rc;
+    if (int rc = flow_arm_settle(s, c.ws, true)) return rc;
     if (int rc = flow_mark_postlaunch(s, c.ws, 0)) return rc;
     c.p = lstm_plan(d, c.head);
     c.lo = lstm_layout(c.p);
@@ -952,12 +983,14 @@
     float* ws = c.ws;
     const int T = d->T, B = d->B, H = d->H, L = d->L;
     unsigned* err = reinterpret_cast<unsigned*>(ws + lo.sync);
-    int* progress = reinterpret_cast<int*>(err) + 8;
-    unsigned* tickets = err + 16;
-    if (!(d->flags & AMDSPEECH_LSTM_ARMED))
+    const bool armed = (d->flags & AMDSPEECH_LSTM_ARMED) != 0;
+    int* progress = reinterpret_cast<int*>(err) + (armed ? FLOW_SYNC_BWD : 8);
+    unsigned* tickets = err + (armed ? FLOW_SYNC_BWD + 8 : 16);
+    if (!armed) {
         if (int rc = flow_fill_bwd_panels(s, d, ws, lo, c.head != nullptr)) return rc;
-    AS_CHECK_HIP(hipMemsetD32Async(reinterpret_cast<hipDeviceptr_t>(progress), T, 8, s));
-    AS_CHECK_HIP(hipMemsetAsync(tickets, 0, 16 * sizeof(unsigned), s));
+        AS_CHECK_HIP(hipMemsetD32Async(reinterpret_cast<hipDeviceptr_t>(progress), T, 8, s));
+        AS_CHECK_HIP(hipMemsetAsync(tickets, 0, 16 * sizeof(unsigned), s));
+    }
 #if FLOW2_CHECK_ORDER
     AS_CHECK_HIP(hipMemsetD32Async(reinterpret_cast<hipDeviceptr_t>(ws + lo.dg), (int)FLOW_SENTINEL, (size_t)L * T * B * 4 * H, s));
     AS_CHECK_HIP(hipMemsetAsync(ws + lo.pdown, 0, (lo.total - lo.pdown) * sizeof(float), s));
@@ -1316,6 +1349,7 @@
         return lstm_fwd(s, two[1]);
     }
     for (FwdCall& c : two) {
+        c.staged = false;
         if (int rc = fwd_prologue(s, c)) return rc;
         if (int rc = fwd_stage(s, c)) return rc;
     }
@@ -1393,6 +1427,23 @@
     if (int rc = check_head(head, false)) return rc;
     return lstm_fwd(static_cast<hipStream_t>(stream), FwdCall{d, static_cast<float*>(ws), kernels, kernel_stride, biases, bias_stride, lengths, h0, c0, head});
 }
+extern "C" int amdspeech_lstm_fwd_in(void* stream, const amdspeech_lstm_desc* d, void* ws, const float* kernels,
+                                     long kernel_stride, const float* biases, long bias_stride, const int* lengths,
+                                     const float* h0, const float* c0, const amdspeech_ctc_head* head, const amdspeech_lstm_input* in) {
+    if (head != nullptr)
+        if (int rc = check_head(head, false)) return rc;
+    AS_CHECK_ARG(in != nullptr, "lstm_fwd_in: null input block");
+    return lstm_fwd(static_cast<hipStream_t>(stream), FwdCall{d, static_cast<float*>(ws), kernels, kernel_stride, biases, bias_stride, lengths, h0, c0, head, in});
+}
+extern "C" int amdspeech_lstm_input_plan(const amdspeech_lstm_desc* d, int C, int U, void* ws, const amdspeech_lstm_input* in) {
+    if (check_desc(d) != AMDSPEECH_OK || ws == nullptr || check_input(d, in) != AMDSPEECH_OK) return -1;
+    amdspeech_ctc_head h{};
+    h.C = C; h.U = U;
+    FwdCall c{d, static_cast<float*>(ws), nullptr, 0, nullptr, 0, nullptr, nullptr, nullptr, nullptr, in};
+    c.p = lstm_plan(d, C > 0 ? &h : nullptr);
+    c.lo = lstm_layout(c.p);
+    return fwd_input_fused(c) ? 1 : 0;
+}
 extern "C" int amdspeech_lstm_bwd_ctc(void* stream, const amdspeech_lstm_desc* d, void* ws, const float* kernels,
                                       long kernel_stride, float* dkernels, float* dbiases, long bias_stride,
                                       const int* lengths, const amdspeech_ctc_head* head) {
diff --git a/rnn-speech_amd/engine.py b/rnn-speech_amd/engine.py
--- a/rnn-speech_amd/engine.py
+++ b/rnn-speech_amd/engine.py
@@ -75,6 +75,7 @@
 
 _BESIDE_FORWARD = os.environ.get("AMDSPEECH_BESIDE_FORWARD", "1") != "0"
 _BESIDE_TAIL = os.environ.get("AMDSPEECH_BESIDE_TAIL", "1") != "0"
+_FUSED_INPUT = os.environ.get("AMDSPEECH_FUSED_INPUT", "1") != "0"
 _BIDIR_PAIR = os.environ.get("AMDSPEECH_BIDIR_PAIR", "1") != "0"
 _FUSED_CTC = os.environ.get("AMDSPEECH_FUSED_CTC", "1") != "0"
 
@@ -219,7 +220,10 @@
         ws = self.lstm_ws.prefix(Tr)
         self._ws, self._Tr = ws, Tr
         ws.set_dropout(keep_in, keep_out, seed)
-        ops.linear_fwd(x[:Tr].view(Tr * B, D), self.p("input_w"), self.p("input_b"), out=ws.z0.view(Tr * B, self.H))
+        lin_in = (x[:Tr].view(Tr * B, D), self.p("input_w"), self.p("input_b"))
+        fuse_in = _FUSED_INPUT and not self.normalization and not self.bidirectional
+        if not fuse_in:
+            ops.linear_fwd(*lin_in, out=ws.z0.view(Tr * B, self.H))
         if self.normalization:
             grp = self._dp_group() if self.sync_batch_norm else None
             if grp is not None and grp.world > 1:
@@ -249,7 +253,7 @@
             ops.lstm_fwd(ws, self.p("kernel_0"), self.layout.kernel_stride, self.p("bias_0"),
                          self.layout.bias_stride, lengths,
                          self.state_h if use_state else None, self.state_c if use_state else None, training=training,
-                         per_diagonal=per_diagonal, head=self._head)
+                         per_diagonal=per_diagonal, head=self._head, input=lin_in if fuse_in else None)
         H = self.H
         if not self.bidirectional:
             if after_lstm is not None:
diff --git a/rnn-speech_amd/lib.py b/rnn-speech_amd/lib.py
--- a/rnn-speech_amd/lib.py
+++ b/rnn-speech_amd/lib.py
@@ -27,6 +27,10 @@
 class CtcHead(C.Structure):
     _fields_ = [("w_out", C.c_void_p), ("b_out", C.c_void_p), ("logits", C.c_void_p), ("dense_labels", C.c_void_p),
                 ("loss", C.c_void_p), ("dlogits", C.c_void_p), ("ctc_ws", C.c_void_p), ("C", C.c_int), ("U", C.c_int)]
+
+
+class LstmInput(C.Structure):
+    _fields_ = [("x", C.c_void_p), ("w", C.c_void_p), ("b", C.c_void_p), ("D", C.c_int)]
 
 
 class LstmPlanInfo(C.Structure):
@@ -157,6 +161,8 @@
     "amdspeech_lstm_bwd_pair": (_I, [_P, C.POINTER(LstmDesc), _P, _P, _P, _P, C.POINTER(LstmDesc), _P, _P, _P, _P, _L, _L, _P]),
     "amdspeech_lstm_fwd_ctc": (_I, [_P, C.POINTER(LstmDesc), _P, _P, _L, _P, _L, _P, _P, _P, C.POINTER(CtcHead)]),
     "amdspeech_lstm_bwd_ctc": (_I, [_P, C.POINTER(LstmDesc), _P, _P, _L, _P, _P, _L, _P, C.POINTER(CtcHead)]),
+    "amdspeech_lstm_fwd_in": (_I, [_P, C.POINTER(LstmDesc), _P, _P, _L, _P, _L, _P, _P, _P, C.POINTER(CtcHead), C.POINTER(LstmInput)]),
+    "amdspeech_lstm_input_plan": (_I, [C.POINTER(LstmDesc), _I, _I, _P, C.POINTER(LstmInput)]),
     "amdspeech_lstm_dropout_multipliers": (_I, [_P, C.POINTER(LstmDesc), _I, _I, _P]),
     "amdspeech_lstm_plan": (_I, [C.POINTER(LstmDesc), _I, _I, C.POINTER(LstmPlanInfo)]),
     "amdspeech_lstm_plan_xw_halves": (_I, [C.POINTER(LstmDesc), _I, _I]),
diff --git a/rnn-speech_amd/ops.py b/rnn-speech_amd/ops.py
--- a/rnn-speech_amd/ops.py
+++ b/rnn-speech_amd/ops.py
@@ -400,9 +400,30 @@
     return n
 
 
-def lstm_fwd(ws, kernels, kernel_stride, biases, bias_stride, lengths, h0=None, c0=None, training=False, per_diagonal=False, head=None):
+def _lstm_input(ws, input):
+    x, w, b = input
+    _chk_f32(x, w, b)
+    if tuple(x.shape) != (ws.T * ws.B, w.shape[0]) or tuple(w.shape) != (x.shape[1], ws.H) or tuple(b.shape) != (ws.H,):
+        raise ValueError("lstm_fwd: input block %r . %r + %r does not give [T*B = %d, H = %d]"
+                         % (tuple(x.shape), tuple(w.shape), tuple(b.shape), ws.T * ws.B, ws.H))
+    return _l.LstmInput(_p(x).value, _p(w).value, _p(b).value, int(x.shape[1]))
+
+
+def lstm_input_fused(ws, input, head=None):
+    c_u = (0, 0) if head is None else ((head.c.C, head.c.U) if isinstance(head, CtcHead) else (int(head[0]), int(head[1])))
+    blk = _lstm_input(ws, input)
+    ws.desc.flags = 0
+    rc = int(ws.lib.amdspeech_lstm_input_plan(C.byref(ws.desc), c_u[0], c_u[1], _p(ws.buf), C.byref(blk)))
+    if rc < 0:
+        raise ValueError("lstm_input_fused: bad arguments")
+    return rc == 1
+
+
+def lstm_fwd(ws, kernels, kernel_stride, biases, bias_stride, lengths, h0=None, c0=None, training=False, per_diagonal=False, head=None,
+             input=None):
     _chk_i32(lengths)
     _chk_f32(h0, c0)
+    blk = _lstm_input(ws, input) if input is not None else None
     root, key = ws._root, (ws.T, int(ws.desc.precision))
     if per_diagonal:
         root._armed, training = None, False
@@ -414,7 +435,11 @@
                      (_l.LSTM_INJECT_TIMEOUT if inject else 0))
     root._fwd_seen = False
     try:
-        if head is None:
+        if blk is not None:
+            _l.check(ws.lib.amdspeech_lstm_fwd_in(_stream(), C.byref(ws.desc), _p(ws.buf), _p(kernels), kernel_stride,
+                                                  _p(biases), bias_stride, _p(lengths), _p(h0), _p(c0),
+                                                  C.byref(head.c) if head is not None else None, C.byref(blk)), "lstm_fwd_in")
+        elif head is None:
             _l.check(ws.lib.amdspeech_lstm_fwd(_stream(), C.byref(ws.desc), _p(ws.buf), _p(kernels), kernel_stride,
                                                _p(biases), bias_stride, _p(lengths), _p(h0), _p(c0)), "lstm_fwd")
         else:
```

New measurement: 2.769 million, median of 6. About the same (+0.8%).
